# toverainc/willow-inference-server

Measured on AMD Instinct MI355X. Metric: realtime_multiple (audio_ms / infer_ms), Whisper large-v2 beam=5, 3.84 s clip, higher is better.
Workload: dtype f16; 1 GPU; whisper-large beam=5 clip=3sec (3840 ms) batch=1/GPU, PCM resident in HBM -> ids on host; parallelism=1 independent replicas (utterance sharding, no data-path collective)

## Files before the change

### willow-inference-server_amd/csrc/dec_kernels.hip

```cpp
#include <string.h>
#include <atomic>
#include <mutex>
#include "common.hpp"
#include "kernels.hpp"

namespace wis {

__global__ void pack_gemv_kernel(const f16* __restrict__ W, f16* __restrict__ Wp, int N, int Npad, int K, int n_scale, float scale, int rows) {
  const int ksteps = K / 32;
  const size_t total = (size_t)Npad * ksteps * 4;
  for (size_t idx = (size_t)blockIdx.x * blockDim.x + threadIdx.x; idx < total; idx += (size_t)gridDim.x * blockDim.x) {
    const int row = (int)(idx % rows);
    size_t t = idx / rows;
    const int kq = (int)(t & 3); t >>= 2;
    const int ks = (int)(t % ksteps), nt = (int)(t / ksteps);
    const int n = rows * nt + row, k = 32 * ks + 8 * kq;
    f16x8 v;
    if (n < N) {
      v = *reinterpret_cast<const f16x8*>(W + (size_t)n * K + k);
      if (n < n_scale) {
#pragma unroll
        for (int j = 0; j < 8; ++j) v[j] = (f16)((float)v[j] * scale);
      }
    } else {
// ... 1945 lines not shown
    if (pub) {
#pragma unroll
      for (int blk = 0; blk < NB; ++blk)
#pragma unroll
        for (int r4 = 0; r4 < 4; ++r4) own[l15][dhb + 16 * blk + r4] = o_[blk][r4];
      if (wave == NKW && kq == 0) { own[l15][64] = Mc; own[l15][65] = Lc; }
    }
    __syncthreads();
    stamp(pf, 5);
    for (int item = tid; item < R * 32; item += NTHR) {
      const int r = item >> 5, dp = item & 31;
      float2 ml[CM], ov[CM];
      unsigned spins = 0;
      for (;;) {
        bool ok = true;
#pragma unroll
        for (int cc = 0; cc < CM - 1; ++cc) {
          if (cc < C - 1) {
            const gran_t* gp = gbase + ((size_t)cc * 8 + r) * 66;
            const gran_t g0 = ld_gran(gp + 64), g1 = ld_gran(gp + 65), g2 = ld_gran(gp + 2 * dp), g3 = ld_gran(gp + 2 * dp + 1);
            ok = ok & ((unsigned)(g0 >> 32) == tag) & ((unsigned)(g1 >> 32) == tag) & ((unsigned)(g2 >> 32) == tag) & ((unsigned)(g3 >> 32) == tag);
            ml[cc] = make_float2(__uint_as_float((unsigned)g0), __uint_as_float((unsigned)g1));
            ov[cc] = make_float2(__uint_as_float((unsigned)g2), __uint_as_float((unsigned)g3));
          }
        }
        if (ok) break;
        if (++spins > CA_SPIN_LIMIT) { atomicOr(epoch, 1u); break; }
        __builtin_amdgcn_s_sleep(1);
      }
      float M_ = own[r][64];
#pragma unroll
      for (int cc = 0; cc < CM - 1; ++cc) if (cc < C - 1) M_ = fmaxf(M_, ml[cc].x);
      float L = 0.f, O0 = 0.f, O1 = 0.f;
#pragma unroll
      for (int cc = 0; cc < CM - 1; ++cc) {
        if (cc < C - 1) {
          const float w = __expf(ml[cc].x - M_);
          L = fmaf(ml[cc].y, w, L); O0 = fmaf(ov[cc].x, w, O0); O1 = fmaf(ov[cc].y, w, O1);
        }
      }
      {
        const float w = __expf(own[r][64] - M_);
        L = fmaf(own[r][65], w, L); O0 = fmaf(own[r][2 * dp], w, O0); O1 = fmaf(own[r][2 * dp + 1], w, O1);
      }
      const float inv = 1.0f / L;
      typedef _Float16 f16x2 __attribute__((ext_vector_type(2)));
      const f16x2 o2 = {(f16)(O0 * inv), (f16)(O1 * inv)};
      *reinterpret_cast<f16x2*>(out + (out_mb ? xf_index(b * R + r, h * 64 + 2 * dp, out_mb) : (size_t)(b * R + r) * d + h * 64 + 2 * dp)) = o2;
    }
    if (tid == 0) __hip_atomic_store(epoch + 1 + b * H + h, tag, __ATOMIC_RELAXED, __HIP_MEMORY_SCOPE_AGENT);
    stamp(pf, 6);
    if (tid == 0) tl_end(prof);
    return;
  }
  float* pbase = part + ((size_t)(b * H + h) * C) * R * 66;
  if (pub) {
    float* pp = pbase + ((size_t)c * R + l15) * 66;
#pragma unroll
    for (int blk = 0; blk < NB; ++blk)
#pragma unroll
      for (int r4 = 0; r4 < 4; ++r4) st_sc1(pp + dhb + 16 * blk + r4, o_[blk][r4]);
    if (wave == NKW && kq == 0) { st_sc1(pp + 64, Mc); st_sc1(pp + 65, Lc); }
  }
  asm volatile("s_waitcnt vmcnt(0)" ::: "memory");
  __syncthreads();
  stamp(pf, 5);
  if (tid == 0) {
    const unsigned prev = __hip_atomic_fetch_add(counters + b * H + h, 1u, __ATOMIC_RELAXED, __HIP_MEMORY_SCOPE_AGENT);
    const int last = (prev == (unsigned)(C - 1));
    if (last) {
      __hip_atomic_store(counters + b * H + h, 0u, __ATOMIC_RELAXED, __HIP_MEMORY_SCOPE_AGENT);
      __builtin_amdgcn_fence(__ATOMIC_ACQUIRE, "agent");
    }
    s_last = last;
  }
  __syncthreads();
  if (tid == 0) tl_end(prof);
  if (!s_last) return;
  for (int item = tid; item < R * 32; item += NTHR) {
    const int r = item >> 5, dp = item & 31;
    float2 ml[CM], ov[CM];
#pragma unroll
    for (int cc = 0; cc < CM; ++cc) {
      if (cc < C) {
        const float* pp = pbase + ((size_t)cc * R + r) * 66;
        ml[cc] = *reinterpret_cast<const float2*>(pp + 64);
        ov[cc] = *reinterpret_cast<const float2*>(pp + 2 * dp);
      }
    }
    float M_ = -INFINITY;
#pragma unroll
    for (int cc = 0; cc < CM; ++cc) if (cc < C) M_ = fmaxf(M_, ml[cc].x);
    float L = 0.f, O0 = 0.f, O1 = 0.f;
#pragma unroll
    for (int cc = 0; cc < CM; ++cc) {
      if (cc < C) {
        const float w = __expf(ml[cc].x - M_);
        L = fmaf(ml[cc].y, w, L); O0 = fmaf(ov[cc].x, w, O0); O1 = fmaf(ov[cc].y, w, O1);
      }
    }
    const float inv = 1.0f / L;
    typedef _Float16 f16x2 __attribute__((ext_vector_type(2)));
    const f16x2 o2 = {(f16)(O0 * inv), (f16)(O1 * inv)};
    *reinterpret_cast<f16x2*>(out + (out_mb ? xf_index(b * R + r, h * 64 + 2 * dp, out_mb) : (size_t)(b * R + r) * d + h * 64 + 2 * dp)) = o2;
  }
  stamp(pf, 6);
}

int launch_dec_cross_attn(hipStream_t st, const float* q, const f16* kx, const f16* vt, f16* out, float* part, unsigned* counters,
                          int B, int R, int H, int d, int T, int Tpad, int chunks, unsigned long long* prof, int out_mb,
                          const float* xres, const float* qcs, const float* qb, unsigned long long* gran, unsigned* epoch, const float* q2, int xres_is_stat, int kv_shared) {
  if (xres && (!qcs || !qb || R > 8 || d > (xres_is_stat ? 2048 : 1280))) { set_error("dec_cross_attn: folded query needs column sums, bias, R <= 8 and d <= 1280 (2048 from partials)"); return WIS_E_ARG; }
  if (xres_is_stat && !xres) { set_error("dec_cross_attn: the fold from partials needs the row partials"); return WIS_E_ARG; }
  if (R < 1 || R > 16 || chunks < 1 || chunks > 16) { set_error("dec_cross_attn: R=%d chunks=%d unsupported", R, chunks); return WIS_E_UNSUPPORTED; }
  if (H > 63 || d > 65535 || T > 65535) { set_error("dec_cross_attn: H=%d d=%d T=%d beyond the packed shape arguments", H, d, T); return WIS_E_UNSUPPORTED; }
  const int CL = cdiv(cdiv(T, chunks), 32) * 32;
  if ((CL != 128 && CL != 256) || CL * chunks > Tpad) { set_error("dec_cross_attn: %d chunks of %d keys unsupported (Tpad %d)", chunks, CL, Tpad); return WIS_E_UNSUPPORTED; }
  const int used = cdiv(T, CL);
  static const int env_spin = getenv("WIS_CA_SPIN") ? atoi(getenv("WIS_CA_SPIN")) : 1;
  const bool spin = env_spin && gran && epoch && B * H <= CA_SPIN_MAX_BH && CL == 256 && used >= 2 && used <= 6 && R <= 8;
  static const int lds_pad = getenv("WIS_CA_LDS_PAD") ? atoi(getenv("WIS_CA_LDS_PAD")) : 0;
  const int shm = (long)B * H * used > 512 ? lds_pad : 0;
#define WIS_CA(TPWv, CMv, FOLDv, SPINv) hipLaunchKernelGGL((dec_cross_attn_kernel<TPWv, CMv, FOLDv, SPINv>), dim3(used, H, B), dim3(256), shm, st, q, kx, vt, xres, q2, epoch, \
                                                  (R | (H << 8) | (CL << 14) | (used << 24)), (d | (T << 16)), (Tpad | (kv_shared ? (1 << 30) : 0)), out, part, counters, prof, out_mb, qcs, qb, gran)
  if (xres_is_stat) {
    const bool small = (long)B * H * used <= 256;
    static const int ca_rs = getenv("WIS_CA_RS") ? atoi(getenv("WIS_CA_RS")) : 2;
    if (ca_rs && (!small || ca_rs >= 2) && CL == 256 && used <= 6 && R <= 8 && d <= 1280) {
#define WIS_CA_RS(SPINv, NTv, NKWv) hipLaunchKernelGGL((dec_cross_attn_rs_kernel<SPINv, NTv, NKWv>), dim3(used, H, B), dim3(128 * NKWv), 0, st, q, kx, vt, xres, q2, epoch, \
                                                        (R | (H << 8) | (CL << 14) | (used << 24)), (d | (T << 16)), (Tpad | (kv_shared ? (1 << 30) : 0)), out, part, counters, prof, out_mb, qcs, qb, gran)
      static const bool rs8 = getenv("WIS_CA_RS8") && atoi(getenv("WIS_CA_RS8")) != 0;
      if (spin) { if (small && rs8) WIS_CA_RS(true, true, 4); else if (small) WIS_CA_RS(true, true, 2); else WIS_CA_RS(true, false, 2); }
      else { if (small && rs8) WIS_CA_RS(false, true, 4); else if (small) WIS_CA_RS(false, true, 2); else WIS_CA_RS(false, false, 2); }
#undef WIS_CA_RS
      return WIS_OK;
    }
    static const bool fold4 = !(getenv("WIS_CA_FOLD4") && atoi(getenv("WIS_CA_FOLD4")) == 0);
    const bool f4 = fold4 && !small && R <= 8;
    if (spin) { if (small) WIS_CA(4, 6, 3, true); else if (f4) WIS_CA(4, 6, 4, true); else WIS_CA(4, 6, 2, true); }
    else if (CL <= 128) WIS_CA(2, 16, 2, false);
    else if (used <= 6) { if (small) WIS_CA(4, 6, 3, false); else if (f4) WIS_CA(4, 6, 4, false); else WIS_CA(4, 6, 2, false); } else WIS_CA(4, 16, 2, false);
  }
  else if (spin) { if (xres) WIS_CA(4, 6, 1, true); else WIS_CA(4, 6, 0, true); }
  else if (xres) { if (CL <= 128) WIS_CA(2, 16, 1, false); else if (used <= 6) WIS_CA(4, 6, 1, false); else WIS_CA(4, 16, 1, false); }
  else { if (CL <= 128) WIS_CA(2, 16, 0, false); else if (used <= 6) WIS_CA(4, 6, 0, false); else WIS_CA(4, 16, 0, false); }
#undef WIS_CA
  return WIS_OK;
}

__device__ __forceinline__ bool better(float av, int ai, float bv, int bi) { return av > bv || (av == bv && ai < bi); }
__device__ __forceinline__ bool better_b(float av, int ai, float bv, int bi) { return (av > bv) | ((av == bv) & (ai < bi)); }
__device__ __forceinline__ void take_better(float& v, int& i, float ov, int oi) { const bool t = better_b(ov, oi, v, i); v = t ? ov : v; i = t ? oi : i; }

template <bool TS>
__global__ __launch_bounds__(256) void logit_stats_kernel(const float* __restrict__ logits, const float* __restrict__ bias_all,
                                                          const float* __restrict__ bias_begin, const int* __restrict__ step_u,
                                                          float* __restrict__ st_max, float* __restrict__ st_sum,
                                                          float* __restrict__ st_val, int* __restrict__ st_idx, SampleCfg cfg,
                                                          int lr_b, int lr_j, int lr_off, unsigned long long* prof, const int* __restrict__ rowmap,
                                                          const int* __restrict__ ts_desc) {
  constexpr int PT = 16;
  const int tid = threadIdx.x, lane = tid & 63, wave = tid >> 6;
  const int sc = blockIdx.x * 4 + wave, m = blockIdx.y, b = m / cfg.beam;
  unsigned long long* pf = (blockIdx.x == 0 && blockIdx.y == 0 && tid == 0) ? prof : nullptr;
  stamp(pf, 0);
  const int step = step_u[b];
  const int SL = cdiv(cfg.n_vocab, STAT_SUB);
  const int lo = sc * SL, hi = (lo + SL < cfg.n_vocab) ? lo + SL : cfg.n_vocab;
  const int jb = m - b * cfg.beam;
  const float* row = logits + (size_t)(b * lr_b + (rowmap ? rowmap[jb] : jb) * lr_j + lr_off) * cfg.n_vocab_pad;
  const bool first = (step == 0) && cfg.suppress_blank;
  const bool mask_eot = cfg.fixed_new > 0 && step < cfg.fixed_new;
  const bool force_eot = cfg.fixed_new > 0 && step >= cfg.fixed_new;

  float vals[PT]; u64 keys[PT];
  float lv[PT], la[PT], lb[PT];
  int r0l = 0, r0h = 0, r1l = 0, r1h = 0, r2l = 0, r2h = 0;
  if constexpr (TS) {
    const int* dsc = ts_desc + m * TS_DESC_INTS;
    r0l = dsc[0]; r0h = dsc[1]; r1l = dsc[2]; r1h = dsc[3]; r2l = dsc[4]; r2h = dsc[5];
  }
#pragma unroll
  for (int i = 0; i < PT; ++i) {
    const int nidx = lo + lane + 64 * i;
    const int cidx = nidx < hi ? nidx : hi - 1;
    lv[i] = row[cidx]; lb[i] = bias_begin[cidx]; la[i] = bias_all ? bias_all[cidx] : 0.f;
  }
  float mx = -INFINITY;
#pragma unroll
  for (int i = 0; i < PT; ++i) {
    const int nidx = lo + lane + 64 * i;
    float v = lv[i] + la[i];
    v = first ? v + lb[i] : v;
    bool dead = (nidx >= hi) | (mask_eot & (nidx == cfg.eot)) | (force_eot & (nidx != cfg.eot));
    if constexpr (TS) dead = dead | ((nidx >= r0l) & (nidx < r0h)) | ((nidx >= r1l) & (nidx < r1h)) | ((nidx >= r2l) & (nidx < r2h));
    v = dead ? -INFINITY : v;
    vals[i] = v; keys[i] = nidx < hi ? sel_key(v, nidx) : 0ull; mx = fmaxf(mx, v);
  }
  stamp(pf, 1);
  mx = wave_max(mx);
  float sum = 0.f;
  if (mx > -INFINITY) {
#pragma unroll
    for (int i = 0; i < PT; ++i) sum += __expf(vals[i] - mx);
  }
  sum = wave_sum(sum);
  if (lane == 0) { st_max[m * STAT_SUB + sc] = mx; st_sum[m * STAT_SUB + sc] = sum; }
  stamp(pf, 2);
  u64 prev = ~0ull;
  for (int rnd = 0; rnd < cfg.n_cand; ++rnd) {
    u64 t[PT];
#pragma unroll
    for (int i = 0; i < PT; ++i) t[i] = keys[i] < prev ? keys[i] : 0ull;
#pragma unroll
    for (int w = PT / 2; w >= 1; w >>= 1)
#pragma unroll
      for (int i = 0; i < w; ++i) t[i] = key_max(t[i], t[i + w]);
    const u64 best = wave_max_key(t[0]);
    if (lane == 0) {
      st_val[((size_t)m * STAT_SUB + sc) * cfg.n_cand + rnd] = best ? key_value(best) : -INFINITY;
      st_idx[((size_t)m * STAT_SUB + sc) * cfg.n_cand + rnd] = best ? key_index(best) : 0x7fffffff;
    }
    prev = best;
  }
  stamp(pf, 3);
}
int launch_logit_stats(hipStream_t st, const float* logits, const float* bias_all, const float* bias_begin, const int* step_u,
                       float* st_max, float* st_sum, float* st_val, int* st_idx, int B, const SampleCfg& cfg, int lr_b, int lr_j, int lr_off,
                       unsigned long long* prof, const int* rowmap, const int* ts_desc) {
  if (cdiv(cfg.n_vocab, STAT_SUB) > 16 * 64) { set_error("logit_stats: vocab too large"); return WIS_E_UNSUPPORTED; }
  if (ts_desc) hipLaunchKernelGGL(logit_stats_kernel<true>, dim3(STAT_SUB / 4, B * cfg.beam), dim3(256), 0, st, logits, bias_all, bias_begin, step_u,
                                  st_max, st_sum, st_val, st_idx, cfg, lr_b, lr_j, lr_off, prof, rowmap, ts_desc);
  else hipLaunchKernelGGL(logit_stats_kernel<false>, dim3(STAT_SUB / 4, B * cfg.beam), dim3(256), 0, st, logits, bias_all, bias_begin, step_u,
                          st_max, st_sum, st_val, st_idx, cfg, lr_b, lr_j, lr_off, prof, rowmap, nullptr);
  return WIS_OK;
}

__device__ __forceinline__ float block_max_256(float v, float* red) {
  v = wave_max(v);
  const int lane = threadIdx.x & 63, wave = threadIdx.x >> 6;
  __syncthreads();
  if (lane == 0) red[wave] = v;
  __syncthreads();
  return fmaxf(fmaxf(red[0], red[1]), fmaxf(red[2], red[3]));
}
__device__ __forceinline__ float block_sum_256(float v, float* red) {
  v = wave_sum(v);
  const int lane = threadIdx.x & 63, wave = threadIdx.x >> 6;
  __syncthreads();
  if (lane == 0) red[wave] = v;
  __syncthreads();
  return (red[0] + red[1]) + (red[2] + red[3]);
}
__global__ __launch_bounds__(256) void ts_rules_kernel(const float* __restrict__ logits, const float* __restrict__ bias_all,
                                                       const float* __restrict__ bias_begin, const int* __restrict__ step_u,
                                                       const int* __restrict__ alive, SampleCfg cfg, int no_ts, int max_init,
                                                       int lr_b, int lr_j, int lr_off, int* __restrict__ ts_desc) {
  __shared__ float red[4];
  const int tid = threadIdx.x, m = blockIdx.x, b = m / cfg.beam, jb = m - b * cfg.beam;
  const int V = cfg.n_vocab, tb = no_ts + 1;
  int step = step_u[b];
  step = step < cfg.max_new ? step : cfg.max_new;
  const bool force_eot = cfg.fixed_new > 0 && step >= cfg.fixed_new;
  int* dsc = ts_desc + m * TS_DESC_INTS;
  if (force_eot) {
    if (tid < TS_DESC_INTS) dsc[tid] = (tid == 7) ? step : 0;
    return;
  }
  const bool first = (step == 0) && cfg.suppress_blank;
  const bool mask_eot = cfg.fixed_new > 0 && step < cfg.fixed_new;
  int r0l = no_ts, r0h = no_ts + 1, r1l = 0, r1h = 0, r2l = 0, r2h = 0;
  if (step == 0) {
    r0l = 0; r0h = tb;
    if (max_init >= 0 && tb + max_init + 1 < V) { r1l = tb + max_init + 1; r1h = V; }
  } else {
    const int* hist = alive + (size_t)m * cfg.max_new;
    const int tk = tid < step ? hist[tid] : -1;
    const float lastpos = block_max_256(tk >= tb ? (float)tid : -1.f, red);
    const int last = hist[step - 1];
    const bool last_ts = last >= tb;
    const bool pen_ts = step < 2 || hist[step - 2] >= tb;
    if (last_ts) { if (pen_ts) { r1l = tb; r1h = V; } else { r1l = 0; r1h = cfg.eot; } }
    if (lastpos >= 0.f) {
      const int t_ts = hist[(int)lastpos];
      const int t_last = (last_ts && !pen_ts) ? t_ts : t_ts + 1;
      r2l = tb; r2h = t_last;
    }
  }
  const float* row = logits + (size_t)(b * lr_b + jb * lr_j + lr_off) * cfg.n_vocab_pad;
  auto value = [&](int i) -> float {
    float v = row[i] + (bias_all ? bias_all[i] : 0.f);
    v = first ? v + bias_begin[i] : v;
    const bool dead = (mask_eot & (i == cfg.eot)) | ((i >= r0l) & (i < r0h)) | ((i >= r1l) & (i < r1h)) | ((i >= r2l) & (i < r2h));
    return dead ? -INFINITY : v;
  };
  float tmx = -INFINITY;
  for (int i = tid; i < tb; i += 256) tmx = fmaxf(tmx, value(i));
  float smx = -INFINITY;
  for (int i = tb + tid; i < V; i += 256) smx = fmaxf(smx, value(i));
  tmx = block_max_256(tmx, red);
  smx = block_max_256(smx, red);
  float ssum = 0.f;
  if (smx > -INFINITY)
    for (int i = tb + tid; i < V; i += 256) ssum += expf(value(i) - smx);
  ssum = block_sum_256(ssum, red);
  const float lse = smx > -INFINITY ? smx + logf(ssum) : -INFINITY;
  const bool ts_wins = lse > tmx;
  if (ts_wins) { r0l = 0; r0h = tb; }
  if (tid == 0) {
    dsc[0] = r0l; dsc[1] = r0h; dsc[2] = r1l; dsc[3] = r1h; dsc[4] = r2l; dsc[5] = r2h; dsc[6] = ts_wins ? 1 : 0; dsc[7] = step;
  }
}
int launch_ts_rules(hipStream_t st, const float* logits, const float* bias_all, const float* bias_begin, const BeamState& bs, int B,
                    const SampleCfg& cfg, int no_ts, int max_init, int lr_b, int lr_j, int lr_off, int* ts_desc) {
  if (cfg.max_new > 256 || no_ts + 1 >= cfg.n_vocab) { set_error("ts_rules: config out of range"); return WIS_E_UNSUPPORTED; }
  hipLaunchKernelGGL(ts_rules_kernel, dim3(B * cfg.beam), dim3(256), 0, st, logits, bias_all, bias_begin, bs.step_u, bs.alive, cfg, no_ts, max_init,
                     lr_b, lr_j, lr_off, ts_desc);
  return WIS_OK;
}

__global__ __launch_bounds__(256) void no_speech_kernel(const float* __restrict__ logits, int ld, int rs, int r0, int V, int ns, float* __restrict__ out) {
  __shared__ float red[4];
  const int b = blockIdx.x, tid = threadIdx.x;
  const float* row = logits + (size_t)(b * rs + r0) * ld;
  float mx = -INFINITY;
  for (int i = tid; i < V; i += 256) mx = fmaxf(mx, row[i]);
  mx = block_max_256(mx, red);
  float s = 0.f;
  for (int i = tid; i < V; i += 256) s += expf(row[i] - mx);
  s = block_sum_256(s, red);
  if (tid == 0) out[b] = expf(row[ns] - mx) / s;
}
int launch_no_speech(hipStream_t st, const float* logits, int ld, int B, int rs, int r0, int V, int ns, float* out) {
  if (ns < 0 || ns >= V) { set_error("no_speech: token %d outside the vocabulary", ns); return WIS_E_ARG; }
  hipLaunchKernelGGL(no_speech_kernel, dim3(B), dim3(256), 0, st, logits, ld, rs, r0, V, ns, out);
  return WIS_OK;
}

__global__ __launch_bounds__(64) void greedy_pick_kernel(const float* __restrict__ st_max, const float* __restrict__ st_sum, const float* __restrict__ st_val,
                                                         const int* __restrict__ st_idx, int n_cand, int V, int* __restrict__ tok_out, float* __restrict__ lp_out) {
  const int m = blockIdx.x, lane = threadIdx.x;
  const float smx = st_max[m * STAT_SUB + lane], ssm = st_sum[m * STAT_SUB + lane];
  const float v = st_val[((size_t)m * STAT_SUB + lane) * n_cand];
  const int ix = st_idx[((size_t)m * STAT_SUB + lane) * n_cand];
  const float M_ = wave_max(smx);
  const float S = wave_sum(smx > -INFINITY ? ssm * __expf(smx - M_) : 0.f);
  const float lse = M_ + logf(S);
  const int tk = ix > V - 1 ? V - 1 : ix;
  const u64 best = wave_max_key(sel_key(v > -INFINITY ? v - lse : -INFINITY, tk));
  if (lane == 0) { tok_out[m] = key_index(best); lp_out[m] = key_value(best); }
}
int launch_greedy_pick(hipStream_t st, const float* st_max, const float* st_sum, const float* st_val, const int* st_idx, int rows, const SampleCfg& cfg, int* tok_out, float* lp_out) {
  hipLaunchKernelGGL(greedy_pick_kernel, dim3(rows), dim3(64), 0, st, st_max, st_sum, st_val, st_idx, cfg.n_cand, cfg.n_vocab, tok_out, lp_out);
  return WIS_OK;
}

__device__ __forceinline__ void publish_step(const BeamState& bs) {
  __threadfence();
  const unsigned B = gridDim.x;
  const unsigned n = atomicAdd(bs.tick, 1u) + 1u;
  if (n % B != 0u) return;
  __threadfence();
  const unsigned steps = n / B;
  const unsigned done = (unsigned)__hip_atomic_load(bs.all_done, __ATOMIC_RELAXED, __HIP_MEMORY_SCOPE_AGENT);
  const unsigned gen = __hip_atomic_load(bs.tick + 1, __ATOMIC_RELAXED, __HIP_MEMORY_SCOPE_AGENT);
  const unsigned gu = bs.giveup ? (__hip_atomic_load(bs.giveup, __ATOMIC_RELAXED, __HIP_MEMORY_SCOPE_AGENT) != 0u ? 1u : 0u) : 0u;
  const unsigned long long now = (unsigned long long)__builtin_amdgcn_s_memrealtime();
  if (steps == 1u) __hip_atomic_store(bs.host + HP_STAMP0, now, __ATOMIC_RELAXED, __HIP_MEMORY_SCOPE_SYSTEM);
  __hip_atomic_store(bs.host + HP_STAMP, now, __ATOMIC_RELAXED, __HIP_MEMORY_SCOPE_SYSTEM);
  if (done >= B && atomicCAS(bs.tick + 2, 0u, steps) == 0u) {
    __hip_atomic_store(bs.host + HP_DONE_STEP, (unsigned long long)steps, __ATOMIC_RELAXED, __HIP_MEMORY_SCOPE_SYSTEM);
    __hip_atomic_store(bs.host + HP_DONE_STAMP, now, __ATOMIC_RELAXED, __HIP_MEMORY_SCOPE_SYSTEM);
  }
  const unsigned long long rec = ((unsigned long long)(gen & 0xFFFFu) << 48) | ((unsigned long long)(steps & 0xFFFFu) << 32) | ((unsigned long long)gu << 16) | (done & 0xFFFFu);
  __hip_atomic_store(bs.host + HP_REC, rec, __ATOMIC_RELEASE, __HIP_MEMORY_SCOPE_SYSTEM);
}

template <int PSL>
__global__ __launch_bounds__(256) void beam_step_kernel(const float* __restrict__ st_max, const float* __restrict__ st_sum,
                                                        const float* __restrict__ st_val, const int* __restrict__ st_idx,
                                                        BeamState bs, RowMeta rm, int P, int ctx, SampleCfg cfg, unsigned long long* prof) {
  constexpr int HPT = (MAX_R * 256 + 255) / 256;
  __shared__ float lse[MAX_R], s_cum[MAX_R];
  __shared__ float cand_v[MAX_CAND]; __shared__ int cand_word[MAX_CAND]; __shared__ int cand_org[MAX_CAND];
  __shared__ int nb_src[MAX_R]; __shared__ int nb_tok[MAX_R]; __shared__ float nb_cum[MAX_R];
  __shared__ int hyp_src[MAX_R]; __shared__ int hyp_slot[MAX_R]; __shared__ int hyp_n[MAX_R]; __shared__ int n_newhyp;
  __shared__ int s_finished;
  __shared__ int sh_alive[MAX_R * 256];
  const int b = blockIdx.x, tid = threadIdx.x, lane = tid & 63, wave = tid >> 6;
  unsigned long long* pf = (b == 0 && tid == 0) ? prof : nullptr;
  stamp(pf, 0);
  const int k = cfg.beam, NC = cfg.n_cand, V = cfg.n_vocab;
  const int r0 = b * k, per_row = STAT_SUB * NC, total = k * per_row;
  float pv_[PSL]; int pi_[PSL];
#pragma unroll
  for (int u = 0; u < PSL; ++u) {
    const int e = tid + 256 * u, ce = e < total ? e : total - 1;
    const float v = st_val[(size_t)r0 * per_row + ce]; const int ix = st_idx[(size_t)r0 * per_row + ce];
    pv_[u] = e < total ? v : -INFINITY; pi_[u] = e < total ? ix : 0x7fffffff;
  }
  float smx[2], ssm[2];
#pragma unroll
  for (int j2 = 0; j2 < 2; ++j2) {
    const int j = wave + 4 * j2, mrow = r0 + (j < k ? j : 0);
    smx[j2] = st_max[mrow * STAT_SUB + lane]; ssm[j2] = st_sum[mrow * STAT_SUB + lane];
  }
  const float my_cum = tid < k ? bs.cum[r0 + tid] : 0.f;
  int hist_tok[HPT];
#pragma unroll
  for (int u = 0; u < HPT; ++u) {
    const int i = tid + 256 * u, j = i >> 8, t = i & 255;
    const int cj = j < k ? j : k - 1, ct = t < cfg.max_new ? t : cfg.max_new - 1;
    hist_tok[u] = bs.alive[(size_t)(r0 + cj) * cfg.max_new + ct];
  }
  const int done_b = bs.done[b];
  const int step = bs.step_u[b];
  const int nh0 = bs.n_hyp[b];
  if (done_b) { if (tid == 0) publish_step(bs); return; }

  stamp(pf, 1);
#pragma unroll
  for (int u = 0; u < HPT; ++u) { const int i = tid + 256 * u; if (i < MAX_R * 256) sh_alive[i] = hist_tok[u]; }
  if (tid < k) s_cum[tid] = my_cum;
#pragma unroll
  for (int j2 = 0; j2 < 2; ++j2) {
    const int j = wave + 4 * j2;
    const float M_ = wave_max(smx[j2]);
    const float S = wave_sum(smx[j2] > -INFINITY ? ssm[j2] * __expf(smx[j2] - M_) : 0.f);
    if (lane == 0 && j < k) lse[j] = M_ + logf(S);
  }
  __syncthreads();
  stamp(pf, 2);
  u64 pk[PSL];
  u64 lbest = 0ull;
  const float inv_per_row = 1.0f / (float)per_row;
#pragma unroll
  for (int u = 0; u < PSL; ++u) {
    const int e = tid + 256 * u;
    int j = (int)(((float)e + 0.5f) * inv_per_row);
    j = j < k ? j : k - 1;
    const float v = pv_[u];
    const float sc_ = (v - lse[j]) + s_cum[j];
    int tk = pi_[u]; tk = tk > V - 1 ? V - 1 : tk;
    pk[u] = e < total ? sel_key(v > -INFINITY ? sc_ : -INFINITY, (j << 20) | tk) : 0ull;
    lbest = key_max(lbest, pk[u]);
  }
  stamp(pf, 3);
  __shared__ u64 wcand[4 * MAX_CAND];
  for (int rnd = 0; rnd < NC; ++rnd) {
    const u64 wb = wave_max_key(lbest);
    if (lane == 0) wcand[wave * NC + rnd] = wb;
#pragma unroll
    for (int u = 0; u < PSL; ++u) pk[u] = pk[u] == wb ? 0ull : pk[u];
    u64 t[PSL];
#pragma unroll
    for (int u = 0; u < PSL; ++u) t[u] = pk[u];
#pragma unroll
    for (int w = PSL / 2; w >= 1; w >>= 1)
#pragma unroll
      for (int u = 0; u < w; ++u) t[u] = key_max(t[u], t[u + w]);
    lbest = t[0];
  }
  if (tid < MAX_CAND) { cand_v[tid] = -INFINITY; cand_word[tid] = V - 1; cand_org[tid] = 0; }
  __syncthreads();
  if (tid < 4 * NC) {
    const u64 mine = wcand[tid];
    int rank = 0;
#pragma unroll
    for (int m2 = 0; m2 < 4 * MAX_CAND; ++m2) rank += (m2 < 4 * NC && wcand[m2] > mine) ? 1 : 0;
    if (mine != 0ull && rank < NC) {
      const int bi = key_index(mine);
      cand_v[rank] = key_value(mine); cand_word[rank] = bi & 0xFFFFF; cand_org[rank] = (bi >> 20) & 0x7FF;
    }
  }
  __syncthreads();

  stamp(pf, 4);
  if (tid == 0) {
    const bool is_last = (step + 1 >= cfg.max_new);
    int nh = nh0, second = k, newh = 0; bool top_finished = false;
    for (int kk = 0; kk < k; ++kk) {
      int next = kk;
      const bool eos = cand_word[kk] == cfg.eot;
      if (eos || is_last) {
        if (kk == 0) top_finished = true;
        if (nh < cfg.max_hyp) {
          hyp_src[newh] = kk; hyp_slot[newh] = nh; hyp_n[newh] = eos ? step : step + 1;
          bs.hyp_score[b * cfg.max_hyp + nh] = cand_v[kk];
          bs.hyp_len[b * cfg.max_hyp + nh] = hyp_n[newh];
          ++newh; ++nh;
        }
        for (int j = second; j < NC; ++j)
          if (cand_word[j] != cfg.eot) { next = j; second = j + 1; break; }
      }
      nb_src[kk] = next; nb_tok[kk] = cand_word[next]; nb_cum[kk] = cand_v[next];
    }
    n_newhyp = newh;
    bs.n_hyp[b] = nh;
    bool fin = is_last;
    if (!fin) fin = cfg.allow_early_exit ? (top_finished && nh >= cfg.early_exit_hyps) : (nh >= cfg.max_candidates);
    s_finished = fin ? 1 : 0;
  }
  __syncthreads();

  stamp(pf, 5);
  const int hist = step;
  const int npos = P - 1 + step + 1;
  for (int hh = 0; hh < n_newhyp; ++hh) {
    const int kk = hyp_src[hh], org = cand_org[kk], n = hyp_n[hh];
    int* dst = bs.hyp_tok + ((size_t)b * cfg.max_hyp + hyp_slot[hh]) * cfg.max_new;
    for (int t = tid; t < n; t += 256) dst[t] = (t < hist) ? sh_alive[org * 256 + t] : cand_word[kk];
  }
  if (s_finished) {
    __syncthreads();
    __threadfence_block();
    if (tid == 0) {
      const int nh = bs.n_hyp[b];
      int best = 0; float bsc = -INFINITY;
      for (int i = 0; i < nh; ++i) {
        float s = bs.hyp_score[b * cfg.max_hyp + i];
        const int n = bs.hyp_len[b * cfg.max_hyp + i];
        if (cfg.length_penalty != 0.f) s /= powf((float)n, cfg.length_penalty);
        if (s > bsc) { bsc = s; best = i; }
      }
      cand_org[0] = best;
      bs.out_len[b] = bs.hyp_len[b * cfg.max_hyp + best];
      bs.out_score[b] = bsc;
      bs.done[b] = 1;
      hp_out_len(bs.host)[b] = bs.hyp_len[b * cfg.max_hyp + best];
      hp_out_score(bs.host)[b] = bsc;
    }
    __syncthreads();
    const int best = cand_org[0], n = bs.hyp_len[b * cfg.max_hyp + best];
    const int* src = bs.hyp_tok + ((size_t)b * cfg.max_hyp + best) * cfg.max_new;
    int* hids = hp_out_ids(bs.host) + (size_t)b * cfg.max_new;
    for (int t = tid; t < n; t += 256) { const int v = src[t]; bs.out_ids[(size_t)b * cfg.max_new + t] = v; hids[t] = v; }
    __threadfence_system();
    __syncthreads();
    if (tid == 0) { atomicAdd(bs.all_done, 1); publish_step(bs); }
    return;
  }
  stamp(pf, 7);
  for (int j = 0; j < k; ++j) {
    const int org = cand_org[nb_src[j]];
    int* al = bs.alive + (size_t)(r0 + j) * cfg.max_new;
    for (int t = tid; t < hist; t += 256) al[t] = sh_alive[org * 256 + t];
    if (tid == 0) {
      al[hist] = nb_tok[j];
      bs.parent[r0 + j] = (step == 0) ? r0 : r0 + org;
      { int* tr = bs.traj + ((size_t)(b * 256 + step) * MAX_R + j) * 2; tr[0] = nb_tok[j]; tr[1] = org; }
      bs.cum[r0 + j] = nb_cum[j];
      rm.tok[r0 + j] = nb_tok[j];
      rm.pos[r0 + j] = npos;
      rm.slot[r0 + j] = r0 + j;
    }
  }
  if (tid == 0) bs.step_u[b] = step + 1;
  __syncthreads();
  if (tid == 0) publish_step(bs);
  stamp(pf, 8);
}
int launch_beam_step(hipStream_t st, const float* st_max, const float* st_sum, const float* st_val, const int* st_idx,
                     const BeamState& bs, const RowMeta& rm, int B, int P, int ctx, const SampleCfg& cfg, unsigned long long* prof) {
  if (cfg.beam > MAX_R || cfg.n_cand > MAX_CAND || cfg.max_new > 256 || ctx > 512 || cfg.n_vocab > (1 << 20)) { set_error("beam_step: config out of range"); return WIS_E_UNSUPPORTED; }
  if (cfg.beam * STAT_SUB * cfg.n_cand <= 16 * 256) hipLaunchKernelGGL(beam_step_kernel<16>, dim3(B), dim3(256), 0, st, st_max, st_sum, st_val, st_idx, bs, rm, P, ctx, cfg, prof);
  else hipLaunchKernelGGL(beam_step_kernel<32>, dim3(B), dim3(256), 0, st, st_max, st_sum, st_val, st_idx, bs, rm, P, ctx, cfg, prof);
  return WIS_OK;
}

constexpr int VS_PERM = 8, VS_BASE = 16, VS_PATH = 32, VS_PATH_W = 32, VS_INTS = VS_PATH + MAX_R * VS_PATH_W;
__global__ __launch_bounds__(64) void draft_match_kernel(BeamState bs, const int* __restrict__ draft, int n_draft, int k, int* __restrict__ vs, int book) {
  __shared__ int org_r[MAX_R], tok_r[MAX_R], perm_prev[MAX_R], old_base[MAX_R], old_path[MAX_R][VS_PATH_W];
  const int tid = threadIdx.x;
  if (bs.done[0]) return;
  const int s = bs.step_u[0] - 1;
  const int t = vs[2];
  if (tid < k) {
    const int* tr = bs.traj + ((size_t)s * MAX_R + tid) * 2;
    tok_r[tid] = tr[0]; org_r[tid] = tr[1]; perm_prev[tid] = vs[VS_PERM + tid]; old_base[tid] = vs[VS_BASE + tid];
  }
  for (int e = tid; e < k * VS_PATH_W; e += 64) old_path[e / VS_PATH_W][e % VS_PATH_W] = vs[VS_PATH + e];
  __syncthreads();
  if (book) {
    for (int e = tid; e < k * VS_PATH_W; e += 64) {
      const int j = e / VS_PATH_W, u = e % VS_PATH_W, pj = org_r[j];
      if (u < t) vs[VS_PATH + e] = old_path[pj][u];
      else if (u == t) vs[VS_PATH + e] = perm_prev[pj];
    }
    if (tid < k) vs[VS_BASE + tid] = old_base[org_r[tid]];
  }
  if (tid == 0) {
    bool ok = s >= 0 && s < n_draft;
    int pn[MAX_R]; unsigned used = 0;
    if (ok) {
      const int* dr = draft + (size_t)s * MAX_R * 2;
      for (int j = 0; j < k && ok; ++j) {
        const int want_org = perm_prev[org_r[j]];
        int hit = -1;
        for (int i = 0; i < k; ++i) if (!((used >> i) & 1u) && dr[2 * i] == tok_r[j] && dr[2 * i + 1] == want_org) { hit = i; break; }
        if (hit < 0) ok = false; else { pn[j] = hit; used |= 1u << hit; }
      }
    }
    if (ok) { for (int j = 0; j < k; ++j) vs[VS_PERM + j] = pn[j]; vs[0] = s + 1; }
    else bs.done[0] = 2;
    if (book) vs[2] = t + 1;
  }
}
int launch_draft_match(hipStream_t st, const BeamState& bs, const int* draft, int n_draft, int beam, int* vstate, int book) {
  hipLaunchKernelGGL(draft_match_kernel, dim3(1), dim3(64), 0, st, bs, draft, n_draft, beam, vstate, book);
  return WIS_OK;
}
__global__ __launch_bounds__(256) void kv_gather_kernel(f16* __restrict__ kc, f16* __restrict__ vc, size_t lstride, const int* __restrict__ vs, const int* __restrict__ done,
                                                        int k, int w0, int ctx, int d) {
  const int lk = blockIdx.y, tid = threadIdx.x;
  const int nwin = vs[2];
  if (done[0] == 1 || nwin <= 0) return;
  f16* cache = ((lk & 1) ? vc : kc) + (size_t)(lk >> 1) * lstride;
  const int c8 = d >> 3, npos = w0 + nwin;
  for (int p = blockIdx.x; p < npos; p += gridDim.x) {
    int par[MAX_R];
#pragma unroll
    for (int j = 0; j < MAX_R; ++j) par[j] = j < k ? (p < w0 ? vs[VS_BASE + j] : vs[VS_PATH + j * VS_PATH_W + (p - w0)]) : j;
    for (int ch = tid; ch < c8; ch += 256) {
      u32x4 v[MAX_R];
#pragma unroll
      for (int j = 0; j < MAX_R; ++j) if (j < k && par[j] != j) v[j] = *reinterpret_cast<const u32x4*>(cache + ((size_t)par[j] * ctx + p) * d + ch * 8);
      asm volatile("s_waitcnt vmcnt(0)" ::: "memory");
#pragma unroll
      for (int j = 0; j < MAX_R; ++j) if (j < k && par[j] != j) *reinterpret_cast<u32x4*>(cache + ((size_t)j * ctx + p) * d + ch * 8) = v[j];
    }
  }
}
int launch_kv_gather(hipStream_t st, f16* kc, f16* vc, size_t layer_stride, int L, const int* vstate, const int* done, int beam, int w0, int ctx, int d) {
  hipLaunchKernelGGL(kv_gather_kernel, dim3(8, 2 * L), dim3(256), 0, st, kc, vc, layer_stride, vstate, done, beam, w0, ctx, d);
  return WIS_OK;
}

__global__ __launch_bounds__(256) void kv_reorder_kernel(f16* __restrict__ kc, f16* __restrict__ vc, size_t lstride, const int* __restrict__ parent,
                                                         const int* __restrict__ step_u, const int* __restrict__ done, int k, int P, int ctx, int d) {
  const int b = blockIdx.z, lk = blockIdx.y, tid = threadIdx.x;
  if (k < 2) return;
  const int r0 = b * k;
  const int dn = done[b], st = step_u[b];
  int par[MAX_R];
#pragma unroll
  for (int j = 0; j < MAX_R; ++j) par[j] = parent[r0 + (j < k ? j : 0)];
  bool ident = true;
#pragma unroll
  for (int j = 0; j < MAX_R; ++j) { if (j < k) ident = ident & (par[j] == r0 + j); else par[j] = r0 + j; }
  if (dn | (int)ident) return;
  const int npos = P - 1 + st;
  f16* cache = ((lk & 1) ? vc : kc) + (size_t)(lk >> 1) * lstride;
  const int c8 = d >> 3;
  for (int p = blockIdx.x; p < npos; p += gridDim.x) {
    for (int ch = tid; ch < c8; ch += 256) {
      u32x4 v[MAX_R];
#pragma unroll
      for (int j = 0; j < MAX_R; ++j) if (j < k && par[j] != r0 + j) v[j] = *reinterpret_cast<const u32x4*>(cache + ((size_t)par[j] * ctx + p) * d + ch * 8);
      asm volatile("s_waitcnt vmcnt(0)" ::: "memory");
#pragma unroll
      for (int j = 0; j < MAX_R; ++j) if (j < k && par[j] != r0 + j) *reinterpret_cast<u32x4*>(cache + ((size_t)(r0 + j) * ctx + p) * d + ch * 8) = v[j];
    }
  }
}
int launch_kv_reorder(hipStream_t st, f16* kc, f16* vc, size_t layer_stride, int L, const BeamState& bs, int B, int beam, int P, int ctx, int d) {
  if (beam < 2) return WIS_OK;
  if (beam > MAX_R) { set_error("kv_reorder: beam %d > %d", beam, MAX_R); return WIS_E_UNSUPPORTED; }
  hipLaunchKernelGGL(kv_reorder_kernel, dim3(8, 2 * L, B), dim3(256), 0, st, kc, vc, layer_stride, bs.parent, bs.step_u, bs.done, beam, P, ctx, d);
  return WIS_OK;
}

__global__ void lang_probs_kernel(const float* __restrict__ logits, int ld, const int* __restrict__ lang_ids, int n_lang, float* __restrict__ probs) {
  const int b = blockIdx.x, lane = threadIdx.x;
  const float* row = logits + (size_t)b * ld;
  float mx = -INFINITY;
  for (int i = lane; i < n_lang; i += 64) mx = fmaxf(mx, row[lang_ids[i]]);
  mx = wave_max(mx);
  float s = 0.f;
  for (int i = lane; i < n_lang; i += 64) s += __expf(row[lang_ids[i]] - mx);
  s = wave_sum(s);
  for (int i = lane; i < n_lang; i += 64) probs[(size_t)b * n_lang + i] = __expf(row[lang_ids[i]] - mx) / s;
}
int launch_lang_probs(hipStream_t st, const float* logits, int ld, const int* lang_ids, int n_lang, float* probs, int B) {
  hipLaunchKernelGGL(lang_probs_kernel, dim3(B), dim3(64), 0, st, logits, ld, lang_ids, n_lang, probs);
  return WIS_OK;
}

}
```

### willow-inference-server_amd/csrc/kernels.hpp

```cpp
#pragma once
#include "common.hpp"

namespace wis {

struct GemmP {
  const f16* A; int64_t a_bs; int a_rs; int a_rpb;
  const f16* W;
  int M, N, K;
  int klen;
  int n_span = 0, n_period = 0, n_phase = 0;
};
static inline GemmP gemm_plain(const f16* A, int lda, const f16* W, int M, int N, int K) {
  GemmP p; p.A = A; p.a_bs = 0; p.a_rs = lda; p.a_rpb = 0x7fffffff; p.W = W; p.M = M; p.N = N; p.K = K; p.klen = 0; return p;
}
int launch_layernorm(hipStream_t st, const float* x, const float* gamma, const float* beta, f16* y, int M, int d);
int launch_gemm_generic(hipStream_t st, const GemmP& p, const float* bias, const float* resid, void* C, int flags);
int launch_gemm_splitk_resid(hipStream_t st, const GemmP& p, int splits, float* scratch, const float* bias, const float* resid, float* X,
                             const float* ln_gamma = nullptr, const float* ln_beta = nullptr, f16* Y = nullptr);
int launch_gemm_conv1(hipStream_t st, const GemmP& p, const float* bias, f16* C, int T);
int launch_gemm_conv2(hipStream_t st, const GemmP& p, const float* bias, const float* pos, float* X, int T);
int launch_gemm_qkv(hipStream_t st, const GemmP& p, const float* bias, f16* qk, f16* vt, int d, int T, int Tpad, int H);
int launch_gemm_crosskv(hipStream_t st, const GemmP& p, const float* bias, f16* kx, f16* vt, int d, int T, int Tpad, int H, int64_t kx_lstride, int64_t vt_lstride);
int launch_enc_attention(hipStream_t st, const f16* qk, const f16* vt, f16* out, int B, int T, int Tpad, int H, float* part = nullptr, unsigned* counters = nullptr,
                         size_t part_cap = 0);
size_t enc_attention_part_floats(int B, int T, int H);
bool enc_attn_lazy();
void launch_scale_q_log2e(hipStream_t st, f16* qk, int64_t rows, int d);

constexpr int MAX_ROWS = 96;
constexpr int MAX_R = 8;
constexpr int MAX_CAND = 2 * MAX_R;
constexpr int MAX_HYP = 3 * MAX_R;

struct RowMeta {
  int* tok;
  int* pos;
  int* slot;
  int* lslot;
};

enum { GV_GELU = 1, GV_RESID = 2, GV_OUT_F32 = 4, GV_LN = 8, GV_QKV = 16,
       GV_LNP = 32,
       GV_LN16 = 64 };
struct GemvP {
  const void* x;
  const float* gamma; const float* beta;
  const float* csum;
  const f16* Wp; const float* bias;
  const float* wscale;
  void* y;
  int M, N, K, flags;
  float* q; f16* kc; f16* vc; const int* slot; const int* pos; int d; int ctx;
  unsigned long long* prof;
  int rows;
  const void* x2; int xsplit;
  f16* y16;
  int xmb;
  const float* stat_in;
  float* stat_out;
  f16* y_xf;
  int ymb;
  int ksplit; float* kpart; unsigned* kcnt;
  int mb0, mbi;
  int wks, wk0;
  unsigned long long* sa_gran; unsigned* sa_epoch; unsigned* sa_flag; f16* sa_out; int sa_rpu, sa_sstride, sa_first;
};
int launch_gemv(hipStream_t st, const GemvP& p);
int launch_gemv_dual(hipStream_t st, const GemvP& pa, const GemvP& pb, const f16* pf_k = nullptr, const f16* pf_v = nullptr, int pf_T = 0, int pf_Tpad = 0, int pf_chunks = 0, int pf_H = 0);
int launch_gemv_frag(hipStream_t st, const GemvP& p);
int launch_gemv_frag3(hipStream_t st, const GemvP* p, int n);
__host__ __device__ static inline size_t xf_index(int m, int k, int MB) {
  return ((size_t)((k >> 5) * MB + (m >> 4)) * 64 + (m & 15) + 16 * ((k >> 3) & 3)) * 8 + (k & 7);
}
int launch_xf_pack(hipStream_t st, const void* x, int x_f16, f16* xf, float* stat, int M, int K, int MB);
int launch_dec_embed_xf(hipStream_t st, const f16* emb, const f16* pos_emb, const int* tok, const int* pos, float* x, f16* xf, float* stat, int M, int d, int MB);
int launch_fold_ln(hipStream_t st, f16* W, const float* gamma, const float* beta, float* bias, float* csum, int N, int K, int n_scale, float qscale);
int launch_csum8(hipStream_t st, const f16* W, const float* scale, float* csum, int N, int K, int n_scale, float qscale);
int launch_pack_gemv8(hipStream_t st, const f16* W, unsigned char* Wp, float* scale, int N, int Npad, int K, int n_scale, float qscale);
int launch_pack_gemv(hipStream_t st, const f16* W, f16* Wp, int N, int Npad, int K, int n_scale, float scale, int rows = 16);
int gemv_rows_for(int N, int K);

int launch_dec_embed(hipStream_t st, const f16* emb, const f16* pos_emb, const int* tok, const int* pos, float* x, int M, int d, f16* xh = nullptr, float* stat = nullptr);
int launch_dec_self_attn(hipStream_t st, const float* q, const f16* kc, const f16* vc, const int* pos, f16* out,
                         int M, int H, int d, int ctx, int rpu, int sstride, int rmul, unsigned long long* prof = nullptr, int out_mb = 0,
                         const int* anc = nullptr, int w0 = 0, int aw = 0, const int* base = nullptr, int nb = 8);
constexpr int CA_SPIN_MAX_BH = 192;
int launch_dec_cross_attn(hipStream_t st, const float* q, const f16* kx, const f16* vt, f16* out, float* part, unsigned* counters,
                          int B, int R, int H, int d, int T, int Tpad, int chunks, unsigned long long* prof = nullptr, int out_mb = 0,
                          const float* xres = nullptr, const float* qcs = nullptr, const float* qb = nullptr,
                          unsigned long long* gran = nullptr, unsigned* epoch = nullptr,
                          const float* q2 = nullptr, int xres_is_stat = 0,
                          int kv_shared = 0);

struct SampleCfg {
  int n_vocab, n_vocab_pad, eot, beam, n_cand, max_new, fixed_new, suppress_blank, greedy;
  float length_penalty; int max_hyp; int allow_early_exit; int max_candidates;
  int early_exit_hyps;
};
#ifndef WIS_EARLY_EXIT_NUM_HYPOTHESES
#define WIS_EARLY_EXIT_NUM_HYPOTHESES 1
#endif
constexpr int STAT_SUB = 64;
int launch_logit_stats(hipStream_t st, const float* logits, const float* bias_all, const float* bias_begin, const int* step_u,
                       float* st_max, float* st_sum, float* st_val, int* st_idx, int B, const SampleCfg& cfg,
                       int lr_b, int lr_j, int lr_off, unsigned long long* prof = nullptr,
                       const int* rowmap = nullptr,
                       const int* ts_desc = nullptr);
constexpr int TS_DESC_INTS = 8;
struct BeamState;
int launch_ts_rules(hipStream_t st, const float* logits, const float* bias_all, const float* bias_begin, const BeamState& bs, int B,
                    const SampleCfg& cfg, int no_ts, int max_init, int lr_b, int lr_j, int lr_off, int* ts_desc);
int launch_no_speech(hipStream_t st, const float* logits, int ld, int B, int rs, int r0, int V, int ns, float* out);
struct BeamState {
  int* step_u;
  int* done;
  int* n_hyp;
  float* cum;
  int* alive;
  int* parent;
  float* hyp_score;
  int* hyp_len;
  int* hyp_tok;
  int* all_done;
  int* out_ids; int* out_len; float* out_score;
  unsigned* tick;
  const unsigned* giveup;
  unsigned long long* host;
  int* traj;
};
enum { HP_REC = 0,
       HP_STAMP0 = 1,
       HP_STAMP = 2,
       HP_DONE_STEP = 3,
       HP_DONE_STAMP = 4,
       HP_WORDS = 8,
       HP_MAXB = MAX_ROWS };
constexpr size_t HP_BYTES = HP_WORDS * 8 + (size_t)HP_MAXB * 8 + (size_t)HP_MAXB * 256 * 4;
__host__ __device__ inline int* hp_out_len(unsigned long long* hp) { return reinterpret_cast<int*>(hp + HP_WORDS); }
__host__ __device__ inline float* hp_out_score(unsigned long long* hp) { return reinterpret_cast<float*>(hp + HP_WORDS) + HP_MAXB; }
__host__ __device__ inline int* hp_out_ids(unsigned long long* hp) { return reinterpret_cast<int*>(hp + HP_WORDS) + 2 * HP_MAXB; }
int launch_kv_reorder(hipStream_t st, f16* kc, f16* vc, size_t layer_stride, int L, const BeamState& bs, int B, int beam, int P, int ctx, int d);
int launch_beam_step(hipStream_t st, const float* st_max, const float* st_sum, const float* st_val, const int* st_idx,
                     const BeamState& bs, const RowMeta& rm, int B, int P, int ctx, const SampleCfg& cfg, unsigned long long* prof = nullptr);
constexpr int DRAFT_VS_INTS = 32 + MAX_R * 32, DRAFT_VS_PERM = 8, DRAFT_VS_BASE = 16;
int launch_draft_match(hipStream_t st, const BeamState& bs, const int* draft, int n_draft, int beam, int* vstate, int book);
int launch_kv_gather(hipStream_t st, f16* kc, f16* vc, size_t layer_stride, int L, const int* vstate, const int* done, int beam, int w0, int ctx, int d);
int launch_greedy_pick(hipStream_t st, const float* st_max, const float* st_sum, const float* st_val, const int* st_idx, int rows, const SampleCfg& cfg, int* tok_out, float* lp_out);
int launch_lang_probs(hipStream_t st, const float* logits, int ld, const int* lang_ids, int n_lang, float* probs, int B);

}
```

### willow-inference-server_amd/csrc/model.hip

```cpp
#include <math.h>
#include <stdlib.h>
#include <string.h>
#include <time.h>
#include <algorithm>
#include <atomic>
#include <chrono>
#include <map>
#include <mutex>
#include <memory>
#include <string>
#include <vector>

#include "common.hpp"
#include "kernels.hpp"

using namespace wis;

namespace wis {

__global__ void convert_kernel(const void* __restrict__ src, int src_f16, void* __restrict__ dst, int dst_f16,
                               int64_t rows, int64_t cols, int64_t dst_ld, int64_t n_scale, float scale) {
  const int64_t total = rows * cols;
  for (int64_t i = (int64_t)blockIdx.x * blockDim.x + threadIdx.x; i < total; i += (int64_t)gridDim.x * blockDim.x) {
    const int64_t r = i / cols, c = i - r * cols;
    float v = src_f16 ? (float)reinterpret_cast<const f16*>(src)[i] : reinterpret_cast<const float*>(src)[i];
    if (r < n_scale) v *= scale;
    if (dst_f16) reinterpret_cast<f16*>(dst)[r * dst_ld + c] = (f16)v; else reinterpret_cast<float*>(dst)[r * dst_ld + c] = v;
  }
}
__global__ void conv_pack_kernel(const void* __restrict__ src, int src_f16, f16* __restrict__ dst, int out, int in, int cpad, int row_len) {
  const int64_t total = (int64_t)out * row_len;
  for (int64_t i = (int64_t)blockIdx.x * blockDim.x + threadIdx.x; i < total; i += (int64_t)gridDim.x * blockDim.x) {
    const int o = (int)(i / row_len), rem = (int)(i - (int64_t)o * row_len), k = rem / cpad, c = rem - k * cpad;
    float v = 0.f;
    if (k < 3 && c < in) {
      const int64_t s = ((int64_t)o * in + c) * 3 + k;
      v = src_f16 ? (float)reinterpret_cast<const f16*>(src)[s] : reinterpret_cast<const float*>(src)[s];
    }
    dst[i] = (f16)v;
  }
}
template <int NM, int CC>
__global__ void mel_to_image_kernel(const float* __restrict__ mel, f16* __restrict__ img) {
  __shared__ float s_t[NM][65];
  const int tid = threadIdx.x, w = blockIdx.y, f0 = blockIdx.x * 64;
  for (int o = tid; o < NM * 64; o += 256) {
    const int m = o >> 6, f = o & 63;
    if (f0 + f < 3000) s_t[m][f] = mel[((size_t)w * NM + m) * 3000 + f0 + f];
  }
  __syncthreads();
  for (int o = tid; o < 64 * CC; o += 256) {
    const int f = o / CC, c = o - f * CC;
    if (f0 + f < 3000) img[((size_t)w * 3002 + f0 + f + 1) * CC + c] = (c < NM) ? (f16)s_t[c][f] : (f16)0.f;
  }
}
static int conv1_k(int n_mels) { return cdiv(3 * conv1_channels(n_mels), 64) * 64; }
__global__ void transpose_to_f16_kernel(const void* __restrict__ src, int src_f16, f16* __restrict__ dst, int rows, int cols) {
  __shared__ float t[32][33];
  const int c0 = blockIdx.x * 32, r0 = blockIdx.y * 32, tx = threadIdx.x & 31, ty = threadIdx.x >> 5;
  for (int i = ty; i < 32; i += 8) {
    const int r = r0 + i, c = c0 + tx;
    if (r < rows && c < cols) t[i][tx] = src_f16 ? (float)reinterpret_cast<const f16*>(src)[(size_t)r * cols + c] : reinterpret_cast<const float*>(src)[(size_t)r * cols + c];
  }
  __syncthreads();
  for (int i = ty; i < 32; i += 8) {
    const int c = c0 + i, r = r0 + tx;
    if (r < rows && c < cols) dst[(size_t)c * rows + r] = (f16)t[tx][i];
  }
}
__global__ void matvec_rows_kernel(const f16* __restrict__ W, int ld, const float* __restrict__ x, float* __restrict__ y, int N, int K) {
  const int n = blockIdx.x, lane = threadIdx.x;
  if (n >= N) return;
  float a = 0.f;
  for (int k = lane; k < K; k += 64) a += (float)W[(size_t)n * ld + k] * x[k];
  a = wave_sum(a);
  if (lane == 0) y[n] = a;
}
__global__ void f16_to_f32_kernel(const f16* __restrict__ s, float* __restrict__ d, int64_t n) {
  for (int64_t i = (int64_t)blockIdx.x * blockDim.x + threadIdx.x; i < n; i += (int64_t)gridDim.x * blockDim.x) d[i] = (float)s[i];
}
}

struct EncLayerW {
  float *ln1_g, *ln1_b, *ln2_g, *ln2_b;
  f16 *w_qkv, *w_out, *w_f1, *w_f2;
  float *b_qkv, *b_out, *b_f1, *b_f2;
};
struct DecLayerW {
  float *ln1_g, *ln1_b, *ln2_g, *ln2_b, *ln3_g, *ln3_b;
  f16 *p_qkv, *p_out, *p_cq, *p_cout, *p_f1, *p_f2;
  f16 *w_ckv;
  float *b_qkv, *b_out, *b_cq, *b_ckv, *b_cout, *b_f1, *b_f2;
  float *s_qkv = nullptr, *s_out = nullptr, *s_cq = nullptr, *s_cout = nullptr, *s_f1 = nullptr, *s_f2 = nullptr;
  float *c_qkv = nullptr, *c_cq = nullptr, *c_f1 = nullptr;
  f16* p_cqo = nullptr; float* b_cqo = nullptr;
};

struct GraphKey {
  int B, beam, P, max_new, fixed_new, suppress_blank, suppress_default, early_exit, spin, sa_nb; float lp, patience;
  int timestamps, max_init;
  bool operator<(const GraphKey& o) const { return memcmp(this, &o, sizeof(GraphKey)) < 0; }
};

struct WeightSlabs {
  int device; std::vector<void*> slabs; size_t bytes = 0;
  ~WeightSlabs() { hipSetDevice(device); for (void* p : slabs) hipFree(p); }
};

struct AlignState {
  std::vector<int> heads;
  bool ready = false;
  bool capture = false;
  int nsel = 0, sel_cap = 0; size_t sel_bytes = 0;
  std::vector<int> layer_s0;
  int* d_sel_head = nullptr; long long* d_koff = nullptr;
  f16* qsel = nullptr;
  float *W = nullptr, *acc = nullptr;
  unsigned* trace = nullptr; int *rev = nullptr, *path = nullptr, *d_meta = nullptr; float* probs = nullptr;
  int cap_ub0 = 0, cap_t0 = 0, cap_P = 0, last_nmax = 0;
  int kv_ub0 = 0;
  hipEvent_t ev[5 + 128] = {}; int n_ev = 0;
  bool ev_partial = false;
};

struct wis_model {
  wis_config_t cfg;
  int device;
  DeviceCtx* ctx;
  hipStream_t st;
  std::shared_ptr<WeightSlabs> wslabs;
  std::vector<void*> allocs;
  char* slab_cur = nullptr; size_t slab_left = 0;
  size_t bytes = 0;
  f16 *w_conv1, *w_conv2; float *b_conv1, *b_conv2, *enc_pos, *enc_ln_g, *enc_ln_b;
  std::vector<EncLayerW> enc;
  std::vector<DecLayerW> dec;
  f16 *emb, *dec_pos, *p_proj; float *dec_ln_g, *dec_ln_b;
  float *bias_all, *bias_begin; int* d_lang_ids;
  int n_vocab_pad;
  int Tpad;
  f16 *img, *c1, *xn, *qk, *vt, *ao, *hbuf, *mem;
  float* x; float* skbuf; float* enc_part = nullptr; unsigned* enc_cnt = nullptr;
  std::vector<f16*> kx, vx;
  std::vector<f16*> kc, vc;
  f16 *kc_all = nullptr, *vc_all = nullptr; size_t kv_layer_stride = 0;
  f16 *kx_all = nullptr, *vx_all = nullptr, *w_ckv_all = nullptr; float* b_ckv_all = nullptr;
  size_t kx_lstride = 0, vx_lstride = 0;
  float *dx, *dq, *logits, *part; f16 *dao, *dh, *dln; unsigned* counters;
  float* dq2 = nullptr;
  int sa_nb = 8;
  float* gf_part = nullptr; unsigned* gf_cnt = nullptr; int gf_ksplit = 1;
  unsigned long long* ca_gran = nullptr; unsigned* ca_epoch = nullptr;
  unsigned long long* sa_gran = nullptr; unsigned* sa_epoch = nullptr;
  bool spin_off = false;
  int handoff_retries = 0;
  bool spin_now = true;
  f16 *dxf = nullptr, *daoxf = nullptr, *dhxf = nullptr; float* dstat = nullptr;
  RowMeta rm; BeamState bs;
  RowMeta rm_win;
  float *st_max, *st_sum, *st_val; int* st_idx;
  int* ts_desc = nullptr;
  float* d_nsp = nullptr;
  int nsp_B = 0;
  float* d_in; int64_t* d_nsamp; float* d_probs;
  int* vstep = nullptr; int* pick_tok = nullptr; float* pick_lp = nullptr;
  int* d_draft = nullptr; int* d_anc = nullptr; int* d_vstate = nullptr; int* d_base = nullptr;
  float* lm_logspec = nullptr; unsigned* lm_gmax = nullptr;
  int* h_pin;
  unsigned long long* h_prog = nullptr;
  unsigned gen = 0;
  int last_B = 0, last_beam = 0;
  bool overrun_left = false;
  hipEvent_t ev[8];
  hipStream_t st_enc = nullptr;
  hipEvent_t ev_enc = nullptr, ev_ckv = nullptr;
  wis_timing_t timing;
  std::map<GraphKey, hipGraphExec_t> graphs;
  bool use_graph;
  float* s_proj = nullptr;
  float* c_proj = nullptr; float* b_proj = nullptr;
  bool w8 = false;
  bool cq_fold = false;
  f16* dxh = nullptr;
  unsigned long long* d_prof;
  bool prof_on; bool prof_all;
  size_t enc_part_cap = 0;
  std::atomic_flag busy = ATOMIC_FLAG_INIT;
  AlignState al;
};

namespace {

constexpr size_t SLAB_BYTES = (size_t)1 << 30;
static int enc_splitk(int d, int M) {
  const int tiles = (d / 128) * cdiv(M, 128);
  if (tiles >= 200) return 0;
  return (tiles <= 128 && (4 * d) % (4 * 64) == 0) ? 4 : 2;
}
template <class T>
int dalloc(wis_model* m, T** p, size_t n_elems) {
  size_t b = n_elems * sizeof(T); if (b == 0) b = 16;
  const size_t align = b >= ((size_t)1 << 20) ? ((size_t)1 << 16) : 256;
  size_t pad = (align - (reinterpret_cast<uintptr_t>(m->slab_cur) & (align - 1))) & (align - 1);
  if (!m->slab_cur || pad + b > m->slab_left) {
    const size_t sb = b > SLAB_BYTES ? ((b + ((size_t)2 << 20) - 1) & ~(((size_t)2 << 20) - 1)) : SLAB_BYTES;
    void* q = nullptr;
    hipError_t e = hipMalloc(&q, sb);
    if (e != hipSuccess) { set_error("hipMalloc(%zu bytes) failed: %s", sb, hipGetErrorString(e)); return WIS_E_NOMEM; }
    m->allocs.push_back(q); m->slab_cur = static_cast<char*>(q); m->slab_left = sb; pad = 0;
  }
  m->slab_cur += pad; m->slab_left -= pad;
  *p = reinterpret_cast<T*>(m->slab_cur);
  m->slab_cur += b; m->slab_left -= b; m->bytes += b + pad;
  return WIS_OK;
}
inline int blocks_for(int64_t n) { int64_t b = (n + 255) / 256; return (int)(b > 8192 ? 8192 : (b < 1 ? 1 : b)); }

struct TensorSrc { const void* p; int f16; int64_t rows, cols; };

struct Loader {
  const wis_tensor_t* t; int n; const char* arena;
  size_t arena_bytes;
  const wis_tensor_t* find(const std::string& name) const {
    for (int i = 0; i < n; ++i) if (name == t[i].name) return &t[i];
    return nullptr;
  }
  int get(const std::string& name, int64_t rows, int64_t cols, TensorSrc* out) const {
    const wis_tensor_t* x = find(name);
    if (!x) { set_error("weight '%s' missing from the index", name.c_str()); return WIS_E_FORMAT; }
    int64_t ne = 1; for (int i = 0; i < x->rank; ++i) ne *= x->shape[i];
    if (ne != rows * cols) { set_error("weight '%s': %lld elements, expected %lld", name.c_str(), (long long)ne, (long long)(rows * cols)); return WIS_E_FORMAT; }
    const size_t es = x->dtype == WIS_DT_F16 ? 2 : 4;
    if (x->dtype != WIS_DT_F16 && x->dtype != WIS_DT_F32) { set_error("weight '%s': dtype %d unsupported", name.c_str(), x->dtype); return WIS_E_FORMAT; }
    if (x->offset + (size_t)ne * es > arena_bytes) { set_error("weight '%s' exceeds the arena", name.c_str()); return WIS_E_FORMAT; }
    out->p = arena + x->offset; out->f16 = x->dtype == WIS_DT_F16; out->rows = rows; out->cols = cols;
    return WIS_OK;
  }
};

int to_f32(wis_model* m, const Loader& L, const std::string& name, int64_t n, float** out, int64_t n_scale = 0, float scale = 1.f) {
  TensorSrc s; WIS_RET(L.get(name, n, 1, &s));
  if (!*out) WIS_RET(dalloc(m, out, (size_t)n));
  hipLaunchKernelGGL(convert_kernel, dim3(blocks_for(n)), dim3(256), 0, m->st, s.p, s.f16, *out, 0, n, (int64_t)1, (int64_t)1, n_scale, scale);
  return WIS_OK;
}
int to_f16_mat(wis_model* m, const Loader& L, const std::string& name, int64_t rows, int64_t cols, f16** out, int64_t n_scale = 0, float scale = 1.f) {
  TensorSrc s; WIS_RET(L.get(name, rows, cols, &s));
  if (!*out) WIS_RET(dalloc(m, out, (size_t)rows * cols));
  hipLaunchKernelGGL(convert_kernel, dim3(blocks_for(rows * cols)), dim3(256), 0, m->st, s.p, s.f16, *out, 1, rows, cols, cols, n_scale, scale);
  return WIS_OK;
}
int to_packed(wis_model* m, const Loader& L, const std::string& name, int N, int K, f16** out, f16* tmp, int n_scale = 0, float scale = 1.f, int* npad_out = nullptr,
              float** scale_out = nullptr, const float* ln_gamma = nullptr, const float* ln_beta = nullptr, float* bias = nullptr, float** csum_out = nullptr) {
  TensorSrc s; WIS_RET(L.get(name, N, K, &s));
  const int rows = gemv_rows_for(N, K);
  const int Npad = cdiv(N, rows) * rows;
  hipLaunchKernelGGL(convert_kernel, dim3(blocks_for((int64_t)N * K)), dim3(256), 0, m->st, s.p, s.f16, tmp, 1, (int64_t)N, (int64_t)K, (int64_t)K, (int64_t)0, 1.f);
  if (ln_gamma) {
    if (!bias || !csum_out) { set_error("to_packed: LayerNorm folding needs a bias vector and a column-sum output"); return WIS_E_ARG; }
    WIS_RET(dalloc(m, csum_out, (size_t)Npad));
    WIS_HIP_CHECK(hipMemsetAsync(*csum_out, 0, (size_t)Npad * 4, m->st));
    WIS_RET(launch_fold_ln(m->st, tmp, ln_gamma, ln_beta, bias, *csum_out, N, K, n_scale, scale));
  }
  if (m->w8 && scale_out) {
    unsigned char* q8 = nullptr;
    WIS_RET(dalloc(m, &q8, (size_t)Npad * K));
    WIS_RET(dalloc(m, scale_out, (size_t)Npad));
    WIS_RET(launch_pack_gemv8(m->st, tmp, q8, *scale_out, N, Npad, K, n_scale, scale));
    if (ln_gamma) WIS_RET(launch_csum8(m->st, tmp, *scale_out, *csum_out, N, K, n_scale, scale));
    *out = reinterpret_cast<f16*>(q8);
  } else {
    WIS_RET(dalloc(m, out, (size_t)Npad * K));
    WIS_RET(launch_pack_gemv(m->st, tmp, *out, N, Npad, K, n_scale, scale, rows));
  }
  if (npad_out) *npad_out = Npad;
  return WIS_OK;
}

int load_weights(wis_model* m, const Loader& L) {
  const wis_config_t& c = m->cfg;
  const int d = c.d_model, V = c.n_vocab;
  const float qs = 0.125f;
  f16* tmp = nullptr;
  f16 *fcat = nullptr, *fwot = nullptr, *fwqo = nullptr;
  {
    size_t big = (size_t)V * d; if ((size_t)4 * d * d > big) big = (size_t)4 * d * d;
    WIS_HIP_CHECK(hipMalloc(reinterpret_cast<void**>(&tmp), big * 2));
    if (m->cq_fold) {
      WIS_HIP_CHECK(hipMalloc(reinterpret_cast<void**>(&fcat), (size_t)2 * d * d * 2));
      WIS_HIP_CHECK(hipMalloc(reinterpret_cast<void**>(&fwot), (size_t)d * d * 2));
      WIS_HIP_CHECK(hipMalloc(reinterpret_cast<void**>(&fwqo), (size_t)d * d * 2));
    }
  }
  int rc = WIS_OK;
  do {
    {
      TensorSrc s;
      if ((rc = L.get("encoder/conv1/weight", d, (int64_t)c.n_mels * 3, &s))) break;
      const int cc = conv1_channels(c.n_mels), k1 = conv1_k(c.n_mels);
      if ((rc = dalloc(m, &m->w_conv1, (size_t)d * k1))) break;
      hipLaunchKernelGGL(conv_pack_kernel, dim3(blocks_for((int64_t)d * k1)), dim3(256), 0, m->st, s.p, s.f16, m->w_conv1, d, c.n_mels, cc, k1);
      if ((rc = L.get("encoder/conv2/weight", d, (int64_t)d * 3, &s))) break;
      if ((rc = dalloc(m, &m->w_conv2, (size_t)d * 3 * d))) break;
      hipLaunchKernelGGL(conv_pack_kernel, dim3(blocks_for((int64_t)d * 3 * d)), dim3(256), 0, m->st, s.p, s.f16, m->w_conv2, d, d, d, 3 * d);
    }
    if ((rc = to_f32(m, L, "encoder/conv1/bias", d, &m->b_conv1))) break;
    if ((rc = to_f32(m, L, "encoder/conv2/bias", d, &m->b_conv2))) break;
    if (L.find("encoder/position_encodings/encodings")) {
      if ((rc = to_f32(m, L, "encoder/position_encodings/encodings", (int64_t)c.n_audio_ctx * d, &m->enc_pos))) break;
    } else {
      std::vector<float> pe((size_t)c.n_audio_ctx * d);
      const int half = d / 2; const double inc = log(10000.0) / (half - 1);
      for (int t = 0; t < c.n_audio_ctx; ++t)
        for (int i = 0; i < half; ++i) {
          const float inv = (float)exp(-inc * i);
          const float a = (float)t * inv;
          pe[(size_t)t * d + i] = sinf(a); pe[(size_t)t * d + half + i] = cosf(a);
        }
      if ((rc = dalloc(m, &m->enc_pos, pe.size()))) break;
      WIS_HIP_CHECK(hipMemcpyAsync(m->enc_pos, pe.data(), pe.size() * 4, hipMemcpyHostToDevice, m->st));
      WIS_HIP_CHECK(hipStreamSynchronize(m->st));
    }
    if ((rc = to_f32(m, L, "encoder/layer_norm/gamma", d, &m->enc_ln_g))) break;
    if ((rc = to_f32(m, L, "encoder/layer_norm/beta", d, &m->enc_ln_b))) break;
    m->enc.resize(c.n_enc_layers);
    for (int l = 0; l < c.n_enc_layers && !rc; ++l) {
      const std::string p = "encoder/layer_" + std::to_string(l) + "/";
      EncLayerW& w = m->enc[l];
      if ((rc = to_f32(m, L, p + "self_attention/layer_norm/gamma", d, &w.ln1_g))) break;
      if ((rc = to_f32(m, L, p + "self_attention/layer_norm/beta", d, &w.ln1_b))) break;
      const float qs_enc = enc_attn_lazy() ? qs * 1.4426950408889634f : qs;
// ... 250 lines not shown
}
int run_cross_kv(wis_model* m, int B) {
  const wis_config_t& c = m->cfg;
  const int d = c.d_model, T = c.n_audio_ctx;
  return launch_gemm_crosskv(m->st, gemm_plain(m->mem, d, m->w_ckv_all, B * T, c.n_dec_layers * 2 * d, d), m->b_ckv_all, m->kx_all, m->vx_all, d, T, m->Tpad,
                             c.n_heads, (int64_t)m->kx_lstride, (int64_t)m->vx_lstride);
}

static int launch_ln_gemv(wis_model* m, hipStream_t st, GemvP g) {
  if (g.M > 8 && (g.flags & GV_LN)) {
    WIS_RET(launch_layernorm(st, reinterpret_cast<const float*>(g.x), nullptr, nullptr, m->dln, g.M, g.K));
    g.x = m->dln; g.csum = nullptr; g.flags &= ~GV_LN;
  }
  return launch_gemv(st, g);
}

static inline void cpu_relax() {
#if !defined(__HIP_DEVICE_COMPILE__) && defined(__x86_64__)
  __builtin_ia32_pause();
#endif
}
static std::atomic<int> g_spin_bh[64];
struct DeferredClaim { hipEvent_t ev; int n; };
static std::mutex g_spin_mu;
static std::vector<DeferredClaim> g_spin_deferred[64];
static void spin_collect(int device) {
  std::lock_guard<std::mutex> lk(g_spin_mu);
  auto& v = g_spin_deferred[device & 63];
  for (size_t i = 0; i < v.size();) {
    if (hipEventQuery(v[i].ev) != hipErrorNotReady) { g_spin_bh[device & 63].fetch_sub(v[i].n, std::memory_order_relaxed); v[i] = v.back(); v.pop_back(); }
    else ++i;
  }
}
struct SpinClaim {
  wis_model* m; int n = 0;
  SpinClaim(wis_model* mm, int B) : m(mm) {
    static const bool env_share = getenv("WIS_CA_SPIN_SHARED") != nullptr;
    m->spin_now = false;
    spin_collect(m->device);
    if (m->spin_off) return;
    if (env_share) { m->spin_now = true; return; }
    const int need = B * m->cfg.n_heads;
    std::atomic<int>& a = g_spin_bh[m->device & 63];
    int cur = a.load(std::memory_order_relaxed);
    while (cur + need <= CA_SPIN_MAX_BH)
      if (a.compare_exchange_weak(cur, cur + need, std::memory_order_relaxed)) { n = need; m->spin_now = true; return; }
  }
  ~SpinClaim() { if (n) g_spin_bh[m->device & 63].fetch_sub(n, std::memory_order_relaxed); }
  void defer(hipStream_t st) {
    if (!n) return;
    if (hipEventRecord(m->ev[6], st) != hipSuccess) return;
    std::lock_guard<std::mutex> lk(g_spin_mu);
    auto& v = g_spin_deferred[m->device & 63];
    for (auto& d : v) if (d.ev == m->ev[6]) { d.n += n; n = 0; return; }
    v.push_back({m->ev[6], n}); n = 0;
  }
  SpinClaim(const SpinClaim&) = delete;
  SpinClaim& operator=(const SpinClaim&) = delete;
};
static int spin_gave_up(wis_model* m, bool* gave_up) {
  int* h = m->h_pin + 2;
  WIS_HIP_CHECK(hipMemcpyAsync(h, m->ca_epoch, 4, hipMemcpyDeviceToHost, m->st));
  WIS_HIP_CHECK(hipStreamSynchronize(m->st));
  *gave_up = *h != 0;
  if (*gave_up) {
    WIS_HIP_CHECK(hipMemsetAsync(m->ca_epoch, 0, 4, m->st));
    m->spin_off = true; ++m->handoff_retries;
    fprintf(stderr, "[wis_hip] device %d: decoder cross-attention granule hand-off timed out; this handle uses the ticket hand-off from now on, the call is repeated\n", m->device);
  }
  return WIS_OK;
}

struct TreeWin { const int* anc; int w0, aw; const int* base = nullptr; };
int align_capture_q(wis_model* m, int l, int M);
constexpr int ANC_W = 32;
static int dec_forward_frag(wis_model* m, int M, int R, int B, bool want_logits, int sstride, int rmul, int chunks, const TreeWin* tw = nullptr) {
  const wis_config_t& c = m->cfg; hipStream_t st = m->st;
  const int d = c.d_model, H = c.n_heads, T = c.n_audio_ctx, ctx = c.n_text_ctx, MB = cdiv(M, 16);
  if (tw && (M % 16 != 0 || R != 16 || B != M / 16)) { set_error("dec_forward_frag: a tree window takes whole groups of 16 rows"); return WIS_E_ARG; }
  WIS_RET(launch_dec_embed_xf(st, m->emb, m->dec_pos, m->rm.tok, m->rm.pos, m->dx, m->dxf, m->dstat, M, d, MB));
  static const bool no_frag_fold = getenv("WIS_NO_FRAG_FOLD") != nullptr;
  const bool fold = m->cq_fold && !no_frag_fold && R <= 8;
  auto base = [&](const void* x, const f16* Wp, const float* wscale, const float* bias, int N, int K, int flags) {
    GemvP g; memset(&g, 0, sizeof(g));
    g.x = x; g.Wp = Wp; g.wscale = wscale; g.bias = bias; g.M = M; g.N = N; g.K = K; g.flags = flags; g.xmb = MB; g.rows = 16;
    return g;
  };
  for (int l = 0; l < c.n_dec_layers; ++l) {
    const DecLayerW& w = m->dec[l];
    unsigned long long* pr = (m->prof_on && l == 0) ? m->d_prof : nullptr;
    GemvP g = base(m->dxf, w.p_qkv, w.s_qkv, w.b_qkv, 3 * d, d, GV_LN | GV_QKV);
    g.csum = w.c_qkv; g.stat_in = m->dstat; g.q = m->dq; g.kc = m->kc[l]; g.vc = m->vc[l]; g.slot = m->rm.slot; g.pos = m->rm.pos; g.d = d; g.ctx = ctx;
    g.prof = pr;
    WIS_RET(launch_gemv_frag(st, g));
    WIS_RET(launch_dec_self_attn(st, m->dq, m->kc[l], m->vc[l], m->rm.pos, m->daoxf, M, H, d, ctx, R, sstride, rmul, nullptr, MB, tw ? tw->anc : nullptr, tw ? tw->w0 : 0, tw ? tw->aw : 0, tw ? tw->base : nullptr, m->sa_nb));
    if (fold) {
      if (m->al.capture) { set_error("dec_forward_frag: an alignment pass needs the un-folded route (more than 8 rows per utterance)"); return WIS_E_STATE; }
      GemvP g3[3];
      g3[0] = base(m->daoxf, w.p_out, nullptr, w.b_out, d, d, GV_RESID);
      g3[0].y = m->dx; g3[0].ymb = MB; g3[0].stat_out = m->dstat; g3[0].prof = pr ? pr + 32 : nullptr;
      g3[1] = base(m->dxf, w.p_cqo, nullptr, w.b_cqo, d, d, GV_OUT_F32);
      g3[1].y = m->dq; g3[1].wks = 2 * d / 32; g3[1].wk0 = 0;
      g3[2] = base(m->daoxf, w.p_cqo, nullptr, nullptr, d, d, GV_OUT_F32);
      g3[2].y = m->dq2; g3[2].wks = 2 * d / 32; g3[2].wk0 = d / 32;
      WIS_RET(launch_gemv_frag3(st, g3, 3));
      WIS_RET(launch_dec_cross_attn(st, m->dq, m->kx[l], m->vx[l], m->daoxf, m->part, m->counters, B, R, H, d, T, m->Tpad, chunks, pr ? pr + 64 : nullptr, MB, m->dstat, w.c_cq, w.b_cq,
                                    m->spin_now ? m->ca_gran : nullptr, m->ca_epoch, m->dq2, 1));
    } else {
    g = base(m->daoxf, w.p_out, w.s_out, w.b_out, d, d, GV_RESID);
    g.y = m->dx; g.y_xf = m->dxf; g.ymb = MB; g.stat_out = m->dstat;
    WIS_RET(launch_gemv_frag(st, g));
    g = base(m->dxf, w.p_cq, w.s_cq, w.b_cq, d, d, GV_LN | GV_OUT_F32);
    g.csum = w.c_cq; g.stat_in = m->dstat; g.y = m->dq;
    WIS_RET(launch_gemv_frag(st, g));
    const size_t ku = (size_t)m->al.kv_ub0 * H * T * 64, vu = (size_t)m->al.kv_ub0 * H * 64 * m->Tpad;
    WIS_RET(launch_dec_cross_attn(st, m->dq, m->kx[l] + ku, m->vx[l] + vu, m->daoxf, m->part, m->counters, B, R, H, d, T, m->Tpad, chunks, nullptr, MB, nullptr, nullptr, nullptr,
                                  (m->spin_now && !tw) ? m->ca_gran : nullptr, m->ca_epoch, nullptr, 0, tw ? 1 : 0));
    if (m->al.capture) WIS_RET(align_capture_q(m, l, M));
    }
    g = base(m->daoxf, w.p_cout, w.s_cout, w.b_cout, d, d, GV_RESID);
    g.y = m->dx; g.y_xf = m->dxf; g.ymb = MB; g.stat_out = m->dstat; g.prof = pr ? pr + 80 : nullptr;
    WIS_RET(launch_gemv_frag(st, g));
    g = base(m->dxf, w.p_f1, w.s_f1, w.b_f1, 4 * d, d, GV_LN | GV_GELU);
    g.csum = w.c_f1; g.stat_in = m->dstat; g.y = m->dhxf; g.ymb = MB; g.prof = pr ? pr + 96 : nullptr;
    WIS_RET(launch_gemv_frag(st, g));
    g = base(m->dhxf, w.p_f2, w.s_f2, w.b_f2, d, 4 * d, GV_RESID);
    g.y = m->dx; g.y_xf = m->dxf; g.ymb = MB; g.stat_out = m->dstat; g.prof = pr ? pr + 112 : nullptr;
    if (m->gf_ksplit > 1 && (4 * d / 32) % (4 * m->gf_ksplit) == 0) { g.ksplit = m->gf_ksplit; g.kpart = m->gf_part; g.kcnt = m->gf_cnt; }
    WIS_RET(launch_gemv_frag(st, g));
  }
  if (want_logits) {
    GemvP g = base(m->dxf, m->p_proj, m->s_proj, m->b_proj, m->n_vocab_pad, d, GV_LN | GV_OUT_F32);
    g.csum = m->c_proj; g.stat_in = m->dstat; g.y = m->logits;
    WIS_RET(launch_gemv_frag(st, g));
  }
  return WIS_OK;
}

static bool sa_fuse_enabled() { const char* e = getenv("WIS_SA_FUSE"); return e && atoi(e) != 0; }
int dec_forward(wis_model* m, int M, int R, int B, bool want_logits, int sstride, int rmul, const TreeWin* tw = nullptr) {
  const wis_config_t& c = m->cfg; hipStream_t st = m->st;
  const int d = c.d_model, H = c.n_heads, T = c.n_audio_ctx, ctx = c.n_text_ctx;
  static const int env_chunks = getenv("WIS_CROSS_CHUNKS") ? atoi(getenv("WIS_CROSS_CHUNKS")) : 0;
  const int chunks = env_chunks ? env_chunks : 6;
  static const bool no_frag = getenv("WIS_NO_FRAG") != nullptr;
  if (tw) return dec_forward_frag(m, M, R, B, want_logits, sstride, rmul, chunks, tw);
  if (M > 8 && !no_frag) return dec_forward_frag(m, M, R, B, want_logits, sstride, rmul, chunks);
  if (m->al.capture) { set_error("wis_align needs the batched-row decoder route (more than 8 rows per pass, WIS_NO_FRAG unset)"); return WIS_E_STATE; }
  const bool fold = m->cq_fold && M <= 8;
  static const int ln_form = [] { const char* e = getenv("WIS_B1_LN"); return !e ? 0 : (!strcmp(e, "f16") ? 2 : (!strcmp(e, "partials") ? 1 : 0)); }();
  const bool ln_ok = fold && d % 64 == 0 && M * (d / 8) <= 13 * 256;
  const bool sa_fuse = m->spin_now && sa_fuse_enabled() && rmul == 1 && M <= 8 && !m->w8 && d % 64 == 0 && ctx >= 64 && !m->prof_on;
  const bool lnp = ln_ok && ln_form == 1 && d <= 1280, ln16 = ln_ok && ln_form == 2 && d <= 2048;
  WIS_RET(launch_dec_embed(st, m->emb, m->dec_pos, m->rm.tok, m->rm.pos, m->dx, M, d, fold ? m->dxh : nullptr, lnp ? m->dstat : nullptr));
  for (int l = 0; l < c.n_dec_layers; ++l) {
    const DecLayerW& w = m->dec[l];
    unsigned long long* pr = (m->prof_on && (l == 0 || m->prof_all)) ? m->d_prof + (size_t)l * 8 * 16 : nullptr;
    GemvP g; memset(&g, 0, sizeof(g));
    g.x = m->dx; g.csum = w.c_qkv; g.Wp = w.p_qkv; g.wscale = w.s_qkv; g.bias = w.b_qkv; g.M = M; g.N = 3 * d; g.K = d;
    g.flags = GV_LN | GV_QKV; g.q = m->dq; g.kc = m->kc[l]; g.vc = m->vc[l]; g.slot = m->rm.slot; g.pos = m->rm.pos; g.d = d; g.ctx = ctx;
    g.prof = pr;
    if (lnp) { g.x = m->dxh; g.stat_in = m->dstat; g.flags = GV_LNP | GV_QKV; }
    if (ln16) { g.x = m->dxh; g.flags = GV_LN16 | GV_QKV; }
    g.rows = gemv_rows_for(g.N == m->n_vocab_pad ? m->cfg.n_vocab : g.N, g.K);
    if (sa_fuse && !lnp && !ln16) { g.sa_gran = m->sa_gran; g.sa_epoch = m->sa_epoch; g.sa_flag = m->ca_epoch; g.sa_out = m->dao; g.sa_rpu = R; g.sa_sstride = sstride; }
    WIS_RET(launch_ln_gemv(m, st, g));
    if (!g.sa_gran) WIS_RET(launch_dec_self_attn(st, m->dq, m->kc[l], m->vc[l], m->rm.pos, m->dao, M, H, d, ctx, R, sstride, rmul, pr ? pr + 16 : nullptr, 0, nullptr, 0, 0, nullptr, m->sa_nb));
    if (fold) {
      GemvP ga; memset(&ga, 0, sizeof(ga));
      ga.x = m->dao; ga.Wp = w.p_out; ga.bias = w.b_out; ga.y = m->dx; ga.M = M; ga.N = d; ga.K = d; ga.flags = GV_RESID; ga.prof = pr ? pr + 32 : nullptr;
      static const bool stat_rows = getenv("WIS_B1_STAT_ROWS") != nullptr;
      if (!stat_rows) ga.stat_out = m->dstat;
      GemvP gb; memset(&gb, 0, sizeof(gb));
      gb.x = m->dxh; gb.x2 = m->dao; gb.xsplit = d; gb.Wp = w.p_cqo; gb.bias = w.b_cqo; gb.y = m->dq; gb.M = M; gb.N = d; gb.K = 2 * d; gb.flags = GV_OUT_F32;
      static const bool ca_pf = getenv("WIS_CA_PREFETCH") && atoi(getenv("WIS_CA_PREFETCH")) != 0;
      if (ca_pf && B == 1) WIS_RET(launch_gemv_dual(st, ga, gb, m->kx[l], m->vx[l], T, m->Tpad, chunks, H));
      else
      WIS_RET(launch_gemv_dual(st, ga, gb));
      if (!stat_rows) WIS_RET(launch_dec_cross_attn(st, m->dq, m->kx[l], m->vx[l], m->dao, m->part, m->counters, B, R, H, d, T, m->Tpad, chunks, pr ? pr + 64 : nullptr, 0,
                                                    m->dstat, w.c_cq, w.b_cq, m->spin_now ? m->ca_gran : nullptr, m->ca_epoch, nullptr, 1));
      else
      WIS_RET(launch_dec_cross_attn(st, m->dq, m->kx[l], m->vx[l], m->dao, m->part, m->counters, B, R, H, d, T, m->Tpad, chunks, pr ? pr + 64 : nullptr, 0,
                                    m->dx, w.c_cq, w.b_cq, m->spin_now ? m->ca_gran : nullptr, m->ca_epoch));
    } else {
    memset(&g, 0, sizeof(g));
    g.x = m->dao; g.Wp = w.p_out; g.wscale = w.s_out; g.bias = w.b_out; g.y = m->dx; g.M = M; g.N = d; g.K = d; g.flags = GV_RESID; g.prof = pr ? pr + 32 : nullptr;
    g.rows = gemv_rows_for(g.N == m->n_vocab_pad ? m->cfg.n_vocab : g.N, g.K);
    WIS_RET(launch_ln_gemv(m, st, g));
    memset(&g, 0, sizeof(g));
    g.x = m->dx; g.csum = w.c_cq; g.Wp = w.p_cq; g.wscale = w.s_cq; g.bias = w.b_cq; g.y = m->dq; g.M = M; g.N = d; g.K = d; g.flags = GV_LN | GV_OUT_F32; g.prof = pr ? pr + 48 : nullptr;
    g.rows = gemv_rows_for(g.N == m->n_vocab_pad ? m->cfg.n_vocab : g.N, g.K);
    WIS_RET(launch_ln_gemv(m, st, g));
    WIS_RET(launch_dec_cross_attn(st, m->dq, m->kx[l], m->vx[l], m->dao, m->part, m->counters, B, R, H, d, T, m->Tpad, chunks, pr ? pr + 64 : nullptr, 0, nullptr, nullptr, nullptr,
                                  m->spin_now ? m->ca_gran : nullptr, m->ca_epoch));
    }
    memset(&g, 0, sizeof(g));
    g.x = m->dao; g.Wp = w.p_cout; g.wscale = w.s_cout; g.bias = w.b_cout; g.y = m->dx; g.M = M; g.N = d; g.K = d; g.flags = GV_RESID; g.prof = pr ? pr + 80 : nullptr;
    if (lnp) { g.y16 = m->dln; g.stat_out = m->dstat; }
    if (ln16) g.y16 = m->dln;
    g.rows = gemv_rows_for(g.N == m->n_vocab_pad ? m->cfg.n_vocab : g.N, g.K);
    WIS_RET(launch_ln_gemv(m, st, g));
    memset(&g, 0, sizeof(g));
    g.x = m->dx; g.csum = w.c_f1; g.Wp = w.p_f1; g.wscale = w.s_f1; g.bias = w.b_f1; g.y = m->dh; g.M = M; g.N = 4 * d; g.K = d; g.flags = GV_LN | GV_GELU; g.prof = pr ? pr + 96 : nullptr;
    if (lnp) { g.x = m->dln; g.stat_in = m->dstat; g.flags = GV_LNP | GV_GELU; }
    if (ln16) { g.x = m->dln; g.flags = GV_LN16 | GV_GELU; }
    g.rows = gemv_rows_for(g.N == m->n_vocab_pad ? m->cfg.n_vocab : g.N, g.K);
    WIS_RET(launch_ln_gemv(m, st, g));
    memset(&g, 0, sizeof(g));
    g.x = m->dh; g.Wp = w.p_f2; g.wscale = w.s_f2; g.bias = w.b_f2; g.y = m->dx; g.M = M; g.N = d; g.K = 4 * d; g.flags = GV_RESID; g.prof = pr ? pr + 112 : nullptr;
    g.y16 = fold ? m->dxh : nullptr;
    if (lnp) g.stat_out = m->dstat;
    g.rows = gemv_rows_for(g.N == m->n_vocab_pad ? m->cfg.n_vocab : g.N, g.K);
    WIS_RET(launch_ln_gemv(m, st, g));
  }
  if (want_logits) {
    GemvP g; memset(&g, 0, sizeof(g));
    g.x = m->dx; g.csum = m->c_proj; g.bias = m->b_proj; g.Wp = m->p_proj; g.wscale = m->s_proj; g.y = m->logits; g.M = M; g.N = m->n_vocab_pad; g.K = d; g.flags = GV_LN | GV_OUT_F32;
    if (lnp) { g.x = m->dxh; g.stat_in = m->dstat; g.flags = GV_LNP | GV_OUT_F32; }
    if (ln16) { g.x = m->dxh; g.flags = GV_LN16 | GV_OUT_F32; }
    g.rows = gemv_rows_for(g.N == m->n_vocab_pad ? m->cfg.n_vocab : g.N, g.K);
    WIS_RET(launch_ln_gemv(m, st, g));
  }
  return WIS_OK;
}

static int init_beam_state(wis_model* m, int B, int beam) {
  hipStream_t st = m->st;
  const int Mrows = B * beam;
  float* cum = reinterpret_cast<float*>(m->h_pin + 2048);
  for (int r = 0; r < Mrows; ++r) cum[r] = (r % beam == 0) ? 0.f : -INFINITY;
  unsigned* tk = reinterpret_cast<unsigned*>(m->h_pin + 2048 + MAX_ROWS);
  m->gen = (m->gen % 0xFFFFu) + 1u;
  tk[0] = 0; tk[1] = m->gen; tk[2] = 0; tk[3] = 0;
  WIS_HIP_CHECK(hipMemcpyAsync(m->bs.cum, cum, (size_t)Mrows * 4, hipMemcpyHostToDevice, st));
  WIS_HIP_CHECK(hipMemcpyAsync(m->bs.tick, tk, 16, hipMemcpyHostToDevice, st));
  WIS_HIP_CHECK(hipMemsetAsync(m->bs.step_u, 0, (size_t)B * 4, st));
  WIS_HIP_CHECK(hipMemsetAsync(m->bs.done, 0, (size_t)B * 4, st));
  WIS_HIP_CHECK(hipMemsetAsync(m->bs.n_hyp, 0, (size_t)B * 4, st));
  WIS_HIP_CHECK(hipMemsetAsync(m->bs.all_done, 0, 16, st));
  WIS_HIP_CHECK(hipMemsetAsync(m->bs.out_len, 0, (size_t)B * 4, st));
  return WIS_OK;
}
static SampleCfg make_sample_cfg(const wis_model* m, const wis_gen_opts_t* o, int beam, int max_new, float* patience_out) {
  const wis_config_t& c = m->cfg;
  SampleCfg sc; memset(&sc, 0, sizeof(sc));
  sc.n_vocab = c.n_vocab; sc.n_vocab_pad = m->n_vocab_pad; sc.eot = c.eot; sc.beam = beam; sc.n_cand = 2 * beam; sc.max_new = max_new;
  sc.fixed_new = o->fixed_new_tokens; sc.suppress_blank = o->suppress_blank; sc.greedy = beam == 1;
  sc.length_penalty = o->length_penalty; sc.max_hyp = MAX_HYP;
  const float patience = o->patience > 0.f ? o->patience : 1.f;
  sc.max_candidates = (int)lroundf((float)beam * patience); if (sc.max_candidates < 1) sc.max_candidates = 1;
  sc.allow_early_exit = (patience == 1.f && o->length_penalty == 0.f) ? 1 : 0;
  sc.early_exit_hyps = WIS_EARLY_EXIT_NUM_HYPOTHESES ? 1 : sc.max_candidates;
  *patience_out = patience;
  return sc;
}

static int check_patience(int beam, float patience) {
  const float p = patience > 0.f ? patience : 1.f;
  const long want = lroundf((float)beam * p);
  if (want > MAX_HYP - beam + 1) {
    set_error("patience %.3g at beam_size %d needs %ld finished hypotheses; the engine holds %d (patience <= %.3g at this beam)", (double)p, beam, want, MAX_HYP - beam + 1,
              (double)(MAX_HYP - beam + 1) / (double)beam);
    return WIS_E_ARG;
  }
  return WIS_OK;
}

int upload_rows(wis_model* m, const std::vector<int>& tok, const std::vector<int>& pos, const std::vector<int>& slot, const std::vector<int>& lslot, bool wait = true, int stage = 1024) {
  const size_t n = tok.size();
  int* h = m->h_pin + stage;
  memcpy(h, tok.data(), n * 4); memcpy(h + MAX_ROWS, pos.data(), n * 4); memcpy(h + 2 * MAX_ROWS, slot.data(), n * 4); memcpy(h + 3 * MAX_ROWS, lslot.data(), n * 4);
  WIS_HIP_CHECK(hipMemcpyAsync(m->rm.tok, h, n * 4, hipMemcpyHostToDevice, m->st));
  WIS_HIP_CHECK(hipMemcpyAsync(m->rm.pos, h + MAX_ROWS, n * 4, hipMemcpyHostToDevice, m->st));
  WIS_HIP_CHECK(hipMemcpyAsync(m->rm.slot, h + 2 * MAX_ROWS, n * 4, hipMemcpyHostToDevice, m->st));
  WIS_HIP_CHECK(hipMemcpyAsync(m->rm.lslot, h + 3 * MAX_ROWS, n * 4, hipMemcpyHostToDevice, m->st));
  if (wait) WIS_HIP_CHECK(hipStreamSynchronize(m->st));
  return WIS_OK;
}

int check_batch(wis_model* m, int B, int beam) {
  if (B < 1 || B > m->cfg.max_batch) { set_error("batch %d outside [1, max_batch=%d]", B, m->cfg.max_batch); return WIS_E_STATE; }
  if (beam < 1 || beam > m->cfg.max_beam || beam > MAX_R) { set_error("beam_size %d outside [1, %d]", beam, m->cfg.max_beam < MAX_R ? m->cfg.max_beam : MAX_R); return WIS_E_STATE; }
  if (B * beam > MAX_ROWS) { set_error("B*beam = %d exceeds %d decoder rows per device batch", B * beam, MAX_ROWS); return WIS_E_STATE; }
  return WIS_OK;
}

static std::atomic<int> g_active_calls[64];
struct BusyGuard {
  wis_model* m; bool ok;
  explicit BusyGuard(wis_model* mm) : m(mm), ok(!mm->busy.test_and_set(std::memory_order_acquire)) { if (ok) g_active_calls[m->device & 63].fetch_add(1, std::memory_order_relaxed); }
  ~BusyGuard() { if (ok) { g_active_calls[m->device & 63].fetch_sub(1, std::memory_order_relaxed); m->busy.clear(std::memory_order_release); } }
};
#define WIS_ENTER(m, what)                                                                                      \
  BusyGuard _busy(m);                                                                                           \
  if (!_busy.ok) { set_error(what ": another call is running on this handle (one call at a time per replica)"); return WIS_E_STATE; }

}

extern "C" {

int wis_version(void) { return WIS_ABI_VERSION; }
const char* wis_last_error(void) { return get_error(); }
int wis_device_count(void) { int n = 0; if (hipGetDeviceCount(&n) != hipSuccess) return 0; return n; }
int wis_supported_compute_types(int device, char* out, size_t cap) {
  (void)device;
  const char* s = "float16,float32,int8_float16";
  if (!out || cap < strlen(s) + 1) { set_error("buffer too small"); return WIS_E_ARG; }
  strcpy(out, s); return WIS_OK;
}

int wis_model_create(const wis_config_t* cfg, const void* arena, size_t arena_bytes, int arena_on_device,
                     const wis_tensor_t* tensors, int n_tensors, int device, wis_model_t** out) {
  if (!cfg || !arena || !tensors || !out || n_tensors <= 0) { set_error("wis_model_create: bad argument"); return WIS_E_ARG; }
  if (cfg->d_model % 128 || cfg->d_model != cfg->n_heads * 64 || cfg->d_model > 2048 || !mel_bins_supported(cfg->n_mels) || cfg->n_enc_layers < 1 || cfg->n_dec_layers < 1 || cfg->n_audio_ctx != 1500 ||
      cfg->n_text_ctx > 512 || cfg->max_batch < 1 || cfg->max_beam < 1 || cfg->max_beam > MAX_R || cfg->n_vocab < 1024) {
    set_error("wis_model_create: unsupported config (d_model %% 128, head_dim 64, n_mels 80 or 128, n_audio_ctx 1500, max_beam <= %d)", MAX_R);
    return WIS_E_UNSUPPORTED;
  }
  DeviceCtx* ctx; WIS_RET(get_ctx(device, &ctx));
  wis_model* m = new wis_model();
  m->cfg = *cfg; m->device = device; m->ctx = ctx;
  m->w8 = cfg->decoder_weight_bits == 8;
  m->cq_fold = !m->w8 && getenv("WIS_NO_CQFOLD") == nullptr;
  m->use_graph = getenv("WIS_NO_GRAPH") == nullptr;
  memset(&m->timing, 0, sizeof(m->timing));
  int rc = WIS_OK;
  void* d_arena = nullptr;
  do {
    if (hipStreamCreateWithFlags(&m->st, hipStreamNonBlocking) != hipSuccess) { set_error("stream create failed"); rc = WIS_E_HIP; break; }
    const char* base = reinterpret_cast<const char*>(arena);
    if (!arena_on_device) {
      if (hipMalloc(&d_arena, arena_bytes) != hipSuccess) { set_error("hipMalloc(arena %zu) failed", arena_bytes); rc = WIS_E_NOMEM; break; }
      if (hipMemcpy(d_arena, arena, arena_bytes, hipMemcpyHostToDevice) != hipSuccess) { set_error("arena upload failed"); rc = WIS_E_HIP; break; }
      base = reinterpret_cast<const char*>(d_arena);
    }
    Loader L{tensors, n_tensors, base, arena_bytes};
    if ((rc = load_weights(m, L))) break;
    {
      std::vector<float> ba(m->n_vocab_pad, 0.f), bb(m->n_vocab_pad, 0.f);
      for (int i = 0; i < cfg->n_suppress; ++i) if (cfg->suppress_ids[i] >= 0 && cfg->suppress_ids[i] < cfg->n_vocab) ba[cfg->suppress_ids[i]] = -INFINITY;
      for (int i = 0; i < cfg->n_suppress_begin; ++i) if (cfg->suppress_ids_begin[i] >= 0 && cfg->suppress_ids_begin[i] < cfg->n_vocab) bb[cfg->suppress_ids_begin[i]] = -INFINITY;
      if ((rc = dalloc(m, &m->bias_all, ba.size())) || (rc = dalloc(m, &m->bias_begin, bb.size()))) break;
      hipMemcpy(m->bias_all, ba.data(), ba.size() * 4, hipMemcpyHostToDevice);
      hipMemcpy(m->bias_begin, bb.data(), bb.size() * 4, hipMemcpyHostToDevice);
      if ((rc = dalloc(m, &m->d_lang_ids, (size_t)(cfg->n_lang > 0 ? cfg->n_lang : 1)))) break;
      if (cfg->n_lang > 0) hipMemcpy(m->d_lang_ids, cfg->lang_ids, (size_t)cfg->n_lang * 4, hipMemcpyHostToDevice);
    }
    m->cfg.suppress_ids = nullptr; m->cfg.suppress_ids_begin = nullptr; m->cfg.lang_ids = nullptr;
    m->wslabs = std::make_shared<WeightSlabs>();
    m->wslabs->device = device; m->wslabs->slabs.swap(m->allocs); m->wslabs->bytes = m->bytes;
    m->slab_cur = nullptr; m->slab_left = 0;
    if ((rc = alloc_buffers(m))) break;
    if (hipStreamSynchronize(m->st) != hipSuccess) { set_error("model init failed"); rc = WIS_E_HIP; break; }
  } while (0);
  if (d_arena) hipFree(d_arena);
  if (rc) { wis_model_destroy(m); return rc; }
  *out = m;
  return WIS_OK;
}

void wis_model_destroy(wis_model_t* m) {
  if (!m) return;
  hipSetDevice(m->device);
  if (m->st) hipStreamSynchronize(m->st);
  spin_collect(m->device);
  for (auto& kv : m->graphs) hipGraphExecDestroy(kv.second);
  for (void* p : m->allocs) hipFree(p);
  if (m->h_pin) hipHostFree(m->h_pin);
  if (m->h_prog) hipHostFree(m->h_prog);
  for (int i = 0; i < 8; ++i) if (m->ev[i]) hipEventDestroy(m->ev[i]);
  for (hipEvent_t e : m->al.ev) if (e) hipEventDestroy(e);
  if (m->st_enc) { hipStreamSynchronize(m->st_enc); hipStreamDestroy(m->st_enc); }
  if (m->ev_enc) hipEventDestroy(m->ev_enc);
  if (m->ev_ckv) hipEventDestroy(m->ev_ckv);
  if (m->st) hipStreamDestroy(m->st);
  delete m;
}
size_t wis_model_device_bytes(const wis_model_t* m) { return m ? m->bytes : 0; }

int wis_model_clone(wis_model_t* parent, wis_model_t** out) {
  if (!parent || !out || !parent->wslabs) { set_error("wis_model_clone: bad argument"); return WIS_E_ARG; }
  WIS_HIP_CHECK(hipSetDevice(parent->device));
  wis_model* m = new wis_model();
  m->cfg = parent->cfg; m->device = parent->device; m->ctx = parent->ctx;
  m->wslabs = parent->wslabs;
  m->w_conv1 = parent->w_conv1; m->w_conv2 = parent->w_conv2; m->b_conv1 = parent->b_conv1; m->b_conv2 = parent->b_conv2;
  m->enc_pos = parent->enc_pos; m->enc_ln_g = parent->enc_ln_g; m->enc_ln_b = parent->enc_ln_b;
  m->enc = parent->enc; m->dec = parent->dec;
  m->emb = parent->emb; m->dec_pos = parent->dec_pos; m->p_proj = parent->p_proj; m->dec_ln_g = parent->dec_ln_g; m->dec_ln_b = parent->dec_ln_b;
  m->bias_all = parent->bias_all; m->bias_begin = parent->bias_begin; m->d_lang_ids = parent->d_lang_ids; m->n_vocab_pad = parent->n_vocab_pad;
  m->w_ckv_all = parent->w_ckv_all; m->b_ckv_all = parent->b_ckv_all;
  m->s_proj = parent->s_proj; m->c_proj = parent->c_proj; m->b_proj = parent->b_proj; m->w8 = parent->w8; m->cq_fold = parent->cq_fold;
  m->use_graph = parent->use_graph;
  m->al.heads = parent->al.heads;
  memset(&m->timing, 0, sizeof(m->timing));
  int rc = WIS_OK;
  do {
    if (hipStreamCreateWithFlags(&m->st, hipStreamNonBlocking) != hipSuccess) { set_error("stream create failed"); rc = WIS_E_HIP; break; }
    if ((rc = alloc_buffers(m))) break;
    if (hipStreamSynchronize(m->st) != hipSuccess) { set_error("clone init failed"); rc = WIS_E_HIP; break; }
  } while (0);
  if (rc) { wis_model_destroy(m); return rc; }
  *out = m;
  return WIS_OK;
}

}

static int fill_tree_window(const int* hd, int s0, int Rw, int k, int P, std::vector<int>& tok, std::vector<int>& pos, std::vector<int>& slot, std::vector<int>& ls, int* ha) {
  const int Mreal = k * Rw, Mpad = cdiv(Mreal, 16) * 16;
  tok.assign(Mpad, 0); pos.assign(Mpad, 0); slot.assign(Mpad, 0); ls.assign(Mpad, 0);
  for (int t = 0; t < Rw; ++t) for (int j = 0; j < k; ++j) {
    const int s_ = s0 + t, r = t * k + j;
    tok[r] = hd[((s_ - 1) * MAX_R + j) * 2]; pos[r] = P - 1 + s_; slot[r] = j; ls[r] = j;
    int a = j;
    for (int sp = s_; sp >= s0; --sp) { ha[r * ANC_W + (sp - s0)] = a; a = hd[((sp - 1) * MAX_R + a) * 2 + 1]; }
    for (int u = t + 1; u < ANC_W; ++u) ha[r * ANC_W + u] = ha[r * ANC_W + t];
  }
  for (int r = Mreal; r < Mpad; ++r) {
    tok[r] = tok[Mreal - 1]; pos[r] = pos[Mreal - 1]; slot[r] = slot[Mreal - 1]; ls[r] = ls[Mreal - 1];
    for (int u = 0; u < ANC_W; ++u) ha[r * ANC_W + u] = ha[(Mreal - 1) * ANC_W + u];
  }
  return Mpad;
}

static int generate_impl(wis_model_t* m, const float* input, int B, const int32_t* prompt, int P,
                 const wis_gen_opts_t* o, int32_t* out_ids, int32_t* out_len, float* out_score, bool* retry,
                 const int32_t* draft = nullptr, int n_draft = 0, int* accepted = nullptr, const int32_t* draft_org = nullptr) {
  *retry = false;
  if (accepted) *accepted = 0;
  m->nsp_B = 0;
  WIS_HIP_CHECK(hipSetDevice(m->device));
  SpinClaim claim(m, B);
  const wis_config_t& c = m->cfg;
  const int beam = o->beam_size < 1 ? 1 : o->beam_size;
  WIS_RET(check_batch(m, B, beam));
  WIS_RET(check_patience(beam, o->patience));
  if (P < 1 || P > 16 || B * P > MAX_ROWS) { set_error("prompt length %d unsupported (1..16, B*P <= %d)", P, MAX_ROWS); return WIS_E_UNSUPPORTED; }
  int max_new = o->max_new_tokens > 0 ? o->max_new_tokens : std::min(c.n_text_ctx / 2, c.n_text_ctx - P);
  if (max_new > 256) max_new = 256;
  if (P - 1 + max_new > c.n_text_ctx) max_new = c.n_text_ctx - (P - 1);
  for (int i = 0; i < B * P; ++i) if (prompt[i] < 0 || prompt[i] >= c.n_vocab) { set_error("prompt token %d out of range", prompt[i]); return WIS_E_ARG; }
  hipStream_t st = m->st;
  const int ctx = c.n_text_ctx;
  auto t0 = std::chrono::steady_clock::now();

  const int Mrows = B * beam;
  WIS_RET(init_beam_state(m, B, beam));
  float patience;
  const SampleCfg sc = make_sample_cfg(m, o, beam, max_new, &patience);
  const float* bias_all = o->suppress_default ? m->bias_all : nullptr;
  const bool drafting = draft != nullptr && n_draft > 0;
  const bool beam_draft = drafting && draft_org != nullptr;
  if (drafting && B != 1) { set_error("wis_generate_draft: one utterance per call (got B = %d)", B); return WIS_E_UNSUPPORTED; }
  if (drafting && !beam_draft && beam != 1) { set_error("wis_generate_draft: beam_size 1 (a beam search is drafted by its trajectory: wis_generate_draft_beam)"); return WIS_E_UNSUPPORTED; }
  const bool ts = o->timestamps != 0;
  const int ts_max_init = o->max_initial_timestamp_index < 0 ? -1 : o->max_initial_timestamp_index;
  if (ts && draft != nullptr) { set_error("timestamps: not available for drafted decodes (wis_generate_draft / wis_generate_draft_beam)"); return WIS_E_UNSUPPORTED; }
  int sot_row = -1;
  if (o->no_speech_prob && !drafting) {
    for (int i = 0; i < P; ++i) if (prompt[i] == c.sot) { sot_row = i; break; }
    for (int b = 1; b < B && sot_row >= 0; ++b) if (prompt[b * P + sot_row] != c.sot) sot_row = -1;
    if (sot_row < 0) { set_error("no_speech_prob: the prompts hold no common <|startoftranscript|> position"); return WIS_E_ARG; }
  }
  if (beam_draft && (beam < 2 || n_draft > 256)) { set_error("wis_generate_draft_beam: beam_size >= 2 and at most 256 draft steps (got %d, %d)", beam, n_draft); return WIS_E_ARG; }
  if (drafting) for (int i = 0; i < n_draft * (beam_draft ? beam : 1); ++i) if (draft[i] < 0 || draft[i] >= c.n_vocab) { set_error("draft token %d out of range", draft[i]); return WIS_E_ARG; }
  if (beam_draft) for (int i = 0; i < n_draft * beam; ++i) if (draft_org[i] < 0 || draft_org[i] >= beam) { set_error("draft origin %d outside [0, beam_size)", draft_org[i]); return WIS_E_ARG; }
  m->last_B = B; m->last_beam = beam;
  const bool spin_call = m->spin_now;
  if (drafting) m->spin_now = false;
  if (!drafting || beam_draft) {
    std::vector<int> tok(B * P), pos(B * P), slot(B * P), ls(B * P);
    for (int b = 0; b < B; ++b) for (int i = 0; i < P; ++i) { tok[b * P + i] = prompt[b * P + i]; pos[b * P + i] = i; slot[b * P + i] = b * beam; ls[b * P + i] = b * beam; }
    WIS_RET(upload_rows(m, tok, pos, slot, ls, false));
  }
  const unsigned long long gen = m->gen;
  if (m->overrun_left) { WIS_HIP_CHECK(hipMemsetAsync(m->ca_epoch, 0, 4, st)); m->overrun_left = false; }
  __atomic_store_n(&m->h_prog[HP_REC], 0ull, __ATOMIC_RELAXED);
  m->h_prog[HP_DONE_STEP] = 0; m->h_prog[HP_DONE_STAMP] = 0; m->h_prog[HP_STAMP0] = 0;

  static const bool one_stream = getenv("WIS_ONE_STREAM") != nullptr;
  static const bool two_streams = getenv("WIS_TWO_STREAMS") != nullptr;
  const bool alone = g_active_calls[m->device & 63].load(std::memory_order_relaxed) <= 1;
  hipStream_t se = (one_stream || !(alone || two_streams)) ? st : m->st_enc;
  if (se != st) WIS_HIP_CHECK(hipStreamWaitEvent(se, m->ev_ckv, 0));
  WIS_HIP_CHECK(hipEventRecord(m->ev[0], se));
  WIS_RET(stage_input(m, input, o->input_kind, B, se));
  WIS_HIP_CHECK(hipEventRecord(m->ev[1], se));
  WIS_RET(run_encoder(m, B, se));
  WIS_HIP_CHECK(hipEventRecord(m->ev[2], se));
  if (se != st) { WIS_HIP_CHECK(hipEventRecord(m->ev_enc, se)); WIS_HIP_CHECK(hipStreamWaitEvent(st, m->ev_enc, 0)); }
  WIS_RET(run_cross_kv(m, B));
  WIS_HIP_CHECK(hipEventRecord(m->ev[3], st));
  WIS_HIP_CHECK(hipEventRecord(m->ev_ckv, st));

  int steps = 1;
  bool spec_done = false;
  bool beam_fin = false;
  std::vector<int> spec_gen; float spec_cum = 0.f; int spec_len = 0;
  if (!drafting) {
    WIS_RET(dec_forward(m, B * P, P, B, true, beam, 0));
    if (sot_row >= 0) WIS_RET(launch_no_speech(st, m->logits, m->n_vocab_pad, B, P, sot_row, c.n_vocab, c.no_speech, m->d_nsp));
    if (ts) WIS_RET(launch_ts_rules(st, m->logits, bias_all, m->bias_begin, m->bs, B, sc, c.no_timestamps, ts_max_init, P, 0, P - 1, m->ts_desc));
    WIS_RET(launch_logit_stats(st, m->logits, bias_all, m->bias_begin, m->bs.step_u, m->st_max, m->st_sum, m->st_val, m->st_idx, B, sc, P, 0, P - 1, WIS_TAPS ? m->d_prof + (size_t)m->cfg.n_dec_layers * 8 * 16 + 16 : nullptr,
                               nullptr, ts ? m->ts_desc : nullptr));
    WIS_RET(launch_beam_step(st, m->st_max, m->st_sum, m->st_val, m->st_idx, m->bs, m->rm, B, P, ctx, sc, WIS_TAPS ? m->d_prof + (size_t)m->cfg.n_dec_layers * 8 * 16 : nullptr));
    WIS_RET(launch_kv_reorder(st, m->kc_all, m->vc_all, m->kv_layer_stride, c.n_dec_layers, m->bs, B, beam, P, ctx, c.d_model));
  } else if (beam_draft) {
    const int k = beam;
    const int nd = std::min(n_draft, max_new - 1);
    int* hd = m->h_pin + 8192;
    for (int s_ = 0; s_ < nd; ++s_) for (int j = 0; j < k; ++j) { hd[(s_ * MAX_R + j) * 2] = draft[s_ * k + j]; hd[(s_ * MAX_R + j) * 2 + 1] = draft_org[s_ * k + j]; }
    int* hv = m->h_pin + 12288;
    for (int i = 0; i < 32; ++i) hv[i] = 0;
    for (int j = 0; j < MAX_R; ++j) { hv[DRAFT_VS_PERM + j] = j; hv[DRAFT_VS_BASE + j] = j; }
    if (nd > 0) WIS_HIP_CHECK(hipMemcpyAsync(m->d_draft, hd, (size_t)nd * MAX_R * 2 * 4, hipMemcpyHostToDevice, st));
    WIS_HIP_CHECK(hipMemcpyAsync(m->d_vstate, hv, 32 * 4, hipMemcpyHostToDevice, st));
    WIS_RET(dec_forward(m, P, P, 1, true, beam, 0));
    WIS_RET(launch_logit_stats(st, m->logits, bias_all, m->bias_begin, m->bs.step_u, m->st_max, m->st_sum, m->st_val, m->st_idx, 1, sc, P, 0, P - 1));
    WIS_RET(launch_beam_step(st, m->st_max, m->st_sum, m->st_val, m->st_idx, m->bs, m->rm, 1, P, ctx, sc));
    WIS_RET(launch_kv_reorder(st, m->kc_all, m->vc_all, m->kv_layer_stride, c.n_dec_layers, m->bs, 1, beam, P, ctx, c.d_model));
    WIS_RET(launch_draft_match(st, m->bs, m->d_draft, nd, k, m->d_vstate, 0));
    const int RW = std::min(ANC_W, MAX_ROWS / k);
    const int s_last = std::min(nd, max_new - 1);
    int* ha = m->h_pin + 12352;
    int* hb = m->h_pin + 15872;
    int* hw2 = m->h_pin + 16000;
    int done_flag = 0, step_dev = 0;
    int pinv[MAX_R];
    for (int j = 0; j < MAX_R; ++j) pinv[j] = j;
    for (int s0 = 1;; ) {
      const int Rw = std::min(RW, s_last - s0 + 1);
      if (Rw >= 1) {
        std::vector<int> tok, pos, slot, ls;
        const int Mpad = fill_tree_window(hd, s0, Rw, k, P, tok, pos, slot, ls, ha);
        for (int r = 0; r < Mpad; ++r) hb[r] = pinv[ha[r * ANC_W]];
        const RowMeta rm_search = m->rm;
        m->rm = m->rm_win;
        int rc = upload_rows(m, tok, pos, slot, ls, false, 15488);
        if (!rc && (hipMemcpyAsync(m->d_anc, ha, (size_t)Mpad * ANC_W * 4, hipMemcpyHostToDevice, st) != hipSuccess ||
                    hipMemcpyAsync(m->d_base, hb, (size_t)Mpad * 4, hipMemcpyHostToDevice, st) != hipSuccess)) { set_error("draft window: ancestor table upload failed"); rc = WIS_E_HIP; }
        TreeWin tw{m->d_anc, P - 1 + s0, ANC_W}; tw.base = m->d_base;
        if (!rc) rc = dec_forward(m, Mpad, 16, Mpad / 16, true, 1, 0, &tw);
        m->rm = rm_search;
        WIS_RET(rc);
        hw2[0] = 0; for (int j = 0; j < MAX_R; ++j) hw2[1 + j] = j;
        WIS_HIP_CHECK(hipMemcpyAsync(m->d_vstate + 2, hw2, 4, hipMemcpyHostToDevice, st));
        WIS_HIP_CHECK(hipMemcpyAsync(m->d_vstate + DRAFT_VS_BASE, hw2 + 1, MAX_R * 4, hipMemcpyHostToDevice, st));
        for (int t = 0; t < Rw; ++t) {
          WIS_RET(launch_logit_stats(st, m->logits, bias_all, m->bias_begin, m->bs.step_u, m->st_max, m->st_sum, m->st_val, m->st_idx, 1, sc, beam, 1, t * k, nullptr, m->d_vstate + DRAFT_VS_PERM));
          WIS_RET(launch_beam_step(st, m->st_max, m->st_sum, m->st_val, m->st_idx, m->bs, m->rm, 1, P, ctx, sc));
          WIS_RET(launch_draft_match(st, m->bs, m->d_draft, nd, k, m->d_vstate, 1));
        }
        WIS_RET(launch_kv_gather(st, m->kc_all, m->vc_all, m->kv_layer_stride, c.n_dec_layers, m->d_vstate, m->bs.done, beam, P - 1 + s0, ctx, c.d_model));
      }
      WIS_HIP_CHECK(hipMemcpyAsync(hv, m->d_vstate, 16 * 4, hipMemcpyDeviceToHost, st));
      WIS_HIP_CHECK(hipMemcpyAsync(hv + 24, m->bs.done, 4, hipMemcpyDeviceToHost, st));
      WIS_HIP_CHECK(hipMemcpyAsync(hv + 25, m->bs.step_u, 4, hipMemcpyDeviceToHost, st));
      WIS_HIP_CHECK(hipStreamSynchronize(st));
      done_flag = hv[24]; step_dev = hv[25];
      if (Rw < 1 || done_flag != 0) break;
      for (int j = 0; j < k; ++j) { const int n_ = hv[DRAFT_VS_PERM + j]; if (n_ >= 0 && n_ < k) pinv[n_] = j; }
      s0 += Rw;
    }
    if (accepted) *accepted = hv[0];
    __atomic_store_n(&m->h_prog[HP_REC], 0ull, __ATOMIC_RELAXED);
    if (done_flag == 1) {
      beam_fin = true; steps = step_dev + 1;
    } else {
      steps = step_dev;
      if (steps < 1) { set_error("wis_generate_draft_beam: verification completed no step"); return WIS_E_STATE; }
      int* hw = m->h_pin + 4096 + 512;
      unsigned* tk = reinterpret_cast<unsigned*>(hw);
      tk[0] = (unsigned)steps; tk[1] = m->gen; tk[2] = 0; tk[3] = 0;
      WIS_HIP_CHECK(hipMemcpyAsync(m->bs.tick, tk, 16, hipMemcpyHostToDevice, st));
      WIS_HIP_CHECK(hipMemsetAsync(m->bs.done, 0, 4, st));
    }
  } else {
    const int nd = std::min(n_draft, max_new - 1);
    std::vector<int> seq(P + nd);
    for (int i = 0; i < P; ++i) seq[i] = prompt[i];
    for (int i = 0; i < nd; ++i) seq[P + i] = draft[i];
    static const int env_rows = getenv("WIS_DRAFT_ROWS") ? atoi(getenv("WIS_DRAFT_ROWS")) : 0;
    const int R = (env_rows >= 16 && env_rows <= MAX_ROWS) ? env_rows / 16 * 16 : MAX_ROWS;
    bool stop = false; int n_acc = 0;
    for (int t0 = 0; t0 < P + nd && !stop; t0 += R) {
      const int rows = std::min(R, P + nd - t0);
      const int f = std::max(P - 1 - t0, 0), nv = rows - f;
      const int Mp = rows > 16 ? cdiv(rows, 16) * 16 : rows;
      std::vector<int> tok(Mp), pos(Mp), slot(Mp, 0), ls(Mp, 0);
      for (int i = 0; i < Mp; ++i) { const int ii = std::min(i, rows - 1); tok[i] = seq[t0 + ii]; pos[i] = t0 + ii; }
      WIS_RET(upload_rows(m, tok, pos, slot, ls));
      if (rows > 16) {
        WIS_HIP_CHECK(hipMemsetAsync(m->d_anc, 0, (size_t)Mp * 16 * 4, st));
        const TreeWin tw{m->d_anc, t0, 16};
        WIS_RET(dec_forward(m, Mp, 16, Mp / 16, nv > 0, 1, 0, &tw));
      } else
      WIS_RET(dec_forward(m, rows, rows, 1, nv > 0, 1, 0));
      if (nv <= 0) continue;
      int* hv = m->h_pin + 4096;
      for (int i = 0; i < nv; ++i) hv[i] = t0 + f + i - (P - 1);
      WIS_HIP_CHECK(hipMemcpyAsync(m->vstep, hv, (size_t)nv * 4, hipMemcpyHostToDevice, st));
      WIS_RET(launch_logit_stats(st, m->logits, bias_all, m->bias_begin, m->vstep, m->st_max, m->st_sum, m->st_val, m->st_idx, nv, sc, 1, 0, f));
      WIS_RET(launch_greedy_pick(st, m->st_max, m->st_sum, m->st_val, m->st_idx, nv, sc, m->pick_tok, m->pick_lp));
      int* ht = m->h_pin + 4096 + MAX_ROWS; float* hl = reinterpret_cast<float*>(m->h_pin + 4096 + 2 * MAX_ROWS);
      WIS_HIP_CHECK(hipMemcpyAsync(ht, m->pick_tok, (size_t)nv * 4, hipMemcpyDeviceToHost, st));
      WIS_HIP_CHECK(hipMemcpyAsync(hl, m->pick_lp, (size_t)nv * 4, hipMemcpyDeviceToHost, st));
      WIS_HIP_CHECK(hipStreamSynchronize(st));
      for (int i = 0; i < nv && !stop; ++i) {
        const int g = hv[i];
        spec_cum = hl[i] + spec_cum;
        spec_gen.push_back(ht[i]);
        const bool eos = ht[i] == c.eot, is_last = g + 1 >= max_new;
        if (eos || is_last) { spec_done = true; spec_len = eos ? g : g + 1; stop = true; }
        else if (g < nd && ht[i] == draft[g]) ++n_acc;
        else stop = true;
      }
    }
    if (accepted) *accepted = n_acc;
    steps = (int)spec_gen.size();
    if (steps < 1) { set_error("wis_generate_draft: verification produced no token"); return WIS_E_STATE; }
    if (!spec_done) {
      int* hs = m->h_pin + 4096;
      for (int t = 0; t < steps; ++t) hs[t] = spec_gen[t];
      WIS_HIP_CHECK(hipMemcpyAsync(m->bs.alive, hs, (size_t)steps * 4, hipMemcpyHostToDevice, st));
      int* hw = m->h_pin + 4096 + 512;
      hw[0] = steps; hw[1] = spec_gen.back(); hw[2] = P - 1 + steps; hw[3] = 0;
      memcpy(hw + 4, &spec_cum, 4);
      WIS_HIP_CHECK(hipMemcpyAsync(m->bs.step_u, hw, 4, hipMemcpyHostToDevice, st));
      WIS_HIP_CHECK(hipMemcpyAsync(m->rm.tok, hw + 1, 4, hipMemcpyHostToDevice, st));
      WIS_HIP_CHECK(hipMemcpyAsync(m->rm.pos, hw + 2, 4, hipMemcpyHostToDevice, st));
      WIS_HIP_CHECK(hipMemcpyAsync(m->rm.slot, hw + 3, 4, hipMemcpyHostToDevice, st));
      WIS_HIP_CHECK(hipMemcpyAsync(m->rm.lslot, hw + 3, 4, hipMemcpyHostToDevice, st));
      WIS_HIP_CHECK(hipMemcpyAsync(m->bs.cum, hw + 4, 4, hipMemcpyHostToDevice, st));
      unsigned* tk = reinterpret_cast<unsigned*>(hw + 8);
      tk[0] = (unsigned)steps; tk[1] = m->gen; tk[2] = 0; tk[3] = 0;
      WIS_HIP_CHECK(hipMemcpyAsync(m->bs.tick, tk, 16, hipMemcpyHostToDevice, st));
    }
  }
  m->spin_now = spin_call;
  WIS_HIP_CHECK(hipEventRecord(m->ev[4], st));
  if (beam_fin) WIS_HIP_CHECK(hipEventRecord(m->ev[5], st));

  auto one_step = [&]() -> int {
    WIS_RET(dec_forward(m, Mrows, beam, B, true, beam, 1));
    if (ts) WIS_RET(launch_ts_rules(st, m->logits, bias_all, m->bias_begin, m->bs, B, sc, c.no_timestamps, ts_max_init, beam, 1, 0, m->ts_desc));
    WIS_RET(launch_logit_stats(st, m->logits, bias_all, m->bias_begin, m->bs.step_u, m->st_max, m->st_sum, m->st_val, m->st_idx, B, sc, beam, 1, 0, WIS_TAPS ? m->d_prof + (size_t)m->cfg.n_dec_layers * 8 * 16 + 16 : nullptr,
                               nullptr, ts ? m->ts_desc : nullptr));
    WIS_RET(launch_beam_step(st, m->st_max, m->st_sum, m->st_val, m->st_idx, m->bs, m->rm, B, P, ctx, sc, WIS_TAPS ? m->d_prof + (size_t)m->cfg.n_dec_layers * 8 * 16 : nullptr));
    WIS_RET(launch_kv_reorder(st, m->kc_all, m->vc_all, m->kv_layer_stride, c.n_dec_layers, m->bs, B, beam, P, ctx, c.d_model));
    return WIS_OK;
  };
  static const bool sa_short = !(getenv("WIS_SA_NB") && atoi(getenv("WIS_SA_NB")) == 0);
  auto nb_for = [&](int passes_done) { const int len = P + passes_done; return !sa_short ? 8 : (len <= 16 ? 2 : (len <= 32 ? 4 : 8)); };
  struct NbReset { wis_model* m; ~NbReset() { m->sa_nb = 8; } } nb_reset{m};
  auto graph_for = [&](int nb, hipGraphExec_t* out) -> int {
    GraphKey key; memset(&key, 0, sizeof(key));
    key.B = B; key.beam = beam; key.P = P; key.max_new = max_new; key.fixed_new = sc.fixed_new; key.suppress_blank = sc.suppress_blank;
    key.suppress_default = o->suppress_default; key.early_exit = sc.allow_early_exit; key.lp = sc.length_penalty; key.patience = patience; key.spin = (m->spin_now ? 1 : 0) | (sa_fuse_enabled() ? 2 : 0);
    key.sa_nb = nb;
    key.timestamps = ts ? 1 : 0; key.max_init = ts ? ts_max_init : 0;
    auto it = m->graphs.find(key);
    if (it != m->graphs.end()) { *out = it->second; return WIS_OK; }
    hipGraph_t graph = nullptr; hipGraphExec_t ge = nullptr;
    WIS_HIP_CHECK(hipStreamBeginCapture(st, hipStreamCaptureModeThreadLocal));
    int rc = one_step();
    hipError_t e = hipStreamEndCapture(st, &graph);
    if (rc) { if (graph) hipGraphDestroy(graph); return rc; }
    if (e != hipSuccess) { set_error("graph capture failed: %s", hipGetErrorString(e)); return WIS_E_HIP; }
    e = hipGraphInstantiate(&ge, graph, nullptr, nullptr, 0);
    hipGraphDestroy(graph);
    if (e != hipSuccess) { set_error("graph instantiate failed: %s", hipGetErrorString(e)); return WIS_E_HIP; }
    m->graphs[key] = ge;
    *out = ge;
    return WIS_OK;
  };
  auto launch_pass = [&](int passes_done) -> int {
    m->sa_nb = nb_for(passes_done);
    if (!m->use_graph) return one_step();
    hipGraphExec_t ge = nullptr;
    WIS_RET(graph_for(m->sa_nb, &ge));
    WIS_HIP_CHECK(hipGraphLaunch(ge, st));
    return WIS_OK;
  };
  int needed = 0;
  bool gave_up = false, from_host = false;
  float decode_ms_dev = -1.f;
  const int known = (sc.fixed_new > 0) ? std::min(max_new, sc.fixed_new + 1) : 0;
  const int limit = known ? known : max_new;
  auto unpack = [&](unsigned long long r, int* st_, int* dn_, int* gu_) {
    if ((r >> 48) != gen) { *st_ = 0; *dn_ = 0; *gu_ = 0; return; }
    *st_ = (int)((r >> 32) & 0xFFFFu); *gu_ = (int)((r >> 16) & 0xFFFFu); *dn_ = (int)(r & 0xFFFFu);
  };
  const int base_done = drafting ? steps : 0;
  const auto t_dec0 = std::chrono::steady_clock::now();
  if (spec_done || beam_fin) {
    needed = steps;
  } else if (known) {
    for (; steps < limit; ++steps) WIS_RET(launch_pass(steps));
    WIS_HIP_CHECK(hipEventRecord(m->ev[5], st));
    WIS_HIP_CHECK(hipStreamSynchronize(st));
    int st_, dn_, gu_; unpack(__atomic_load_n(&m->h_prog[HP_REC], __ATOMIC_ACQUIRE), &st_, &dn_, &gu_);
    gave_up = gu_ != 0;
    if (!gave_up && dn_ < B) { set_error("decode did not terminate within %d steps (done %d of %d)", steps, dn_, B); return WIS_E_STATE; }
    needed = steps;
  } else {
    const int depth = o->queue_depth > 0 ? o->queue_depth : 2;
    auto t_last = std::chrono::steady_clock::now();
    int seen = -1, st_ = 0, dn_ = 0, gu_ = 0;
    static const bool trace = getenv("WIS_EOT_TRACE") != nullptr;
    struct Tr { int step; unsigned long long dev; double host_us; int launched; };
    std::vector<Tr> tr;
    const auto t_loop = std::chrono::steady_clock::now();
    for (unsigned spins = 0;; ++spins) {
      unpack(__atomic_load_n(&m->h_prog[HP_REC], __ATOMIC_ACQUIRE), &st_, &dn_, &gu_);
      if (st_ < base_done) st_ = base_done;
      if (dn_ >= B || gu_) break;
      if (st_ >= limit) break;
      if (steps < limit && steps - st_ < depth) {
        const auto tl0 = std::chrono::steady_clock::now();
        WIS_RET(launch_pass(steps));
        ++steps;
        if (trace) tr.push_back({-steps, 0ull, std::chrono::duration<double, std::micro>(std::chrono::steady_clock::now() - tl0).count(), steps});
        continue;
      }
      if (st_ != seen) {
        seen = st_; t_last = std::chrono::steady_clock::now(); spins = 0;
        if (trace) tr.push_back({st_, m->h_prog[HP_STAMP], std::chrono::duration<double, std::micro>(t_last - t_loop).count(), steps});
      }
      else if ((spins & 1023u) == 1023u) {
        const double idle = std::chrono::duration<double>(std::chrono::steady_clock::now() - t_last).count();
        if (idle > 30.0) { set_error("decode made no progress for 30 s (step %d of %d enqueued)", st_, steps); return WIS_E_HIP; }
        if (idle > 200e-6) { struct timespec ts = {0, 20000}; nanosleep(&ts, nullptr); }
      }
      cpu_relax();
    }
    if (trace) {
      unsigned long long prev_dev = 0;
      for (size_t i = 0; i < tr.size(); ++i) {
        if (tr[i].step < 0) { fprintf(stderr, "[eot-trace]   launch of step %d took the host %.1f us\n", -tr[i].step, tr[i].host_us); continue; }
        fprintf(stderr, "[eot-trace] step %d seen by the host at %.1f us (device clock +%.1f us since the previous record), %d steps enqueued\n", tr[i].step, tr[i].host_us,
                prev_dev ? (double)(tr[i].dev - prev_dev) * 0.01 : 0.0, tr[i].launched);
        prev_dev = tr[i].dev;
      }
      fprintf(stderr, "[eot-trace] done seen at %.1f us: %d of %d utterances, %d steps enqueued\n", std::chrono::duration<double, std::micro>(std::chrono::steady_clock::now() - t_loop).count(), dn_, B, steps);
    }
    gave_up = gu_ != 0;
    if (!gave_up && dn_ < B) { set_error("decode did not terminate within %d steps (done %d of %d)", steps, dn_, B); return WIS_E_STATE; }
    if (!gave_up) {
      from_host = true;
      needed = (int)m->h_prog[HP_DONE_STEP];
      const unsigned long long s0 = m->h_prog[HP_STAMP0], s1 = m->h_prog[HP_DONE_STAMP];
      decode_ms_dev = s1 > s0 ? (float)((double)(s1 - s0) * 1e-5) : 0.f;
      if (drafting) decode_ms_dev = std::chrono::duration<float, std::milli>(std::chrono::steady_clock::now() - t_dec0).count();
    }
  }
  if (gave_up) {
    WIS_HIP_CHECK(hipMemsetAsync(m->ca_epoch, 0, 4, st));
    WIS_HIP_CHECK(hipStreamSynchronize(st));
    m->spin_off = true; *retry = true; ++m->handoff_retries;
    fprintf(stderr, "[wis_hip] device %d: decoder cross-attention granule hand-off timed out; this handle uses the ticket hand-off from now on, the call is repeated\n", m->device);
    return WIS_OK;
  }
  if (spec_done) {
    float sfin = spec_cum;
    if (sc.length_penalty != 0.f) sfin /= powf((float)spec_len, sc.length_penalty);
    out_len[0] = spec_len;
    for (int t = 0; t < max_new; ++t) out_ids[t] = t < spec_len ? spec_gen[t] : 0;
    if (out_score) out_score[0] = sfin;
    from_host = true; decode_ms_dev = 0.f;
  } else if (from_host) {
    const int* hl = hp_out_len(m->h_prog); const float* hs = hp_out_score(m->h_prog); const int* hi = hp_out_ids(m->h_prog);
    for (int b = 0; b < B; ++b) {
      int n = hl[b];
      if (n < 0 || n > max_new) { set_error("decode result of utterance %d has length %d outside [0, %d]", b, n, max_new); return WIS_E_STATE; }
      out_len[b] = n;
      for (int t = 0; t < max_new; ++t) out_ids[(size_t)b * max_new + t] = t < n ? hi[(size_t)b * max_new + t] : 0;
      if (out_score) out_score[b] = hs[b];
    }
  } else {
    std::vector<int32_t> ids((size_t)B * 256);
    WIS_HIP_CHECK(hipMemcpyAsync(ids.data(), m->bs.out_ids, (size_t)B * 256 * 4, hipMemcpyDeviceToHost, st));
    WIS_HIP_CHECK(hipMemcpyAsync(out_len, m->bs.out_len, (size_t)B * 4, hipMemcpyDeviceToHost, st));
    std::vector<float> sc_h(B);
    WIS_HIP_CHECK(hipMemcpyAsync(sc_h.data(), m->bs.out_score, (size_t)B * 4, hipMemcpyDeviceToHost, st));
    WIS_HIP_CHECK(hipStreamSynchronize(st));
    for (int b = 0; b < B; ++b) {
      if (out_len[b] > max_new) out_len[b] = max_new;
      for (int t = 0; t < max_new; ++t) out_ids[(size_t)b * max_new + t] = t < out_len[b] ? ids[(size_t)b * max_new + t] : 0;
      if (out_score) out_score[b] = sc_h[b];
    }
  }
  auto t1 = std::chrono::steady_clock::now();
  float ms;
  hipEventElapsedTime(&ms, m->ev[0], m->ev[1]); m->timing.logmel_ms = ms;
  hipEventElapsedTime(&ms, m->ev[1], m->ev[2]); m->timing.encoder_ms = ms;
  hipEventElapsedTime(&ms, m->ev[2], m->ev[3]); m->timing.crosskv_ms = ms;
  hipEventElapsedTime(&ms, m->ev[3], m->ev[4]); m->timing.prefill_ms = ms;
  if (from_host) m->timing.decode_ms = decode_ms_dev; else { hipEventElapsedTime(&ms, m->ev[4], m->ev[5]); m->timing.decode_ms = ms; }
  m->timing.total_ms = std::chrono::duration<float, std::milli>(t1 - t0).count();
  m->timing.decode_steps = steps;
  m->timing.decode_steps_needed = needed;
  if (steps > needed) { claim.defer(st); m->overrun_left = true; }
  if (sot_row >= 0) m->nsp_B = B;
  return WIS_OK;
}

extern "C" {

int wis_generate(wis_model_t* m, const float* input, int B, const int32_t* prompt, int P,
                 const wis_gen_opts_t* o, int32_t* out_ids, int32_t* out_len, float* out_score) {
  if (!m || !input || !prompt || !o || !out_ids || !out_len) { set_error("wis_generate: bad argument"); return WIS_E_ARG; }
  WIS_ENTER(m, "wis_generate")
  bool retry = false;
  WIS_RET(generate_impl(m, input, B, prompt, P, o, out_ids, out_len, out_score, &retry));
  if (retry) {
    WIS_RET(generate_impl(m, input, B, prompt, P, o, out_ids, out_len, out_score, &retry));
    if (retry) { set_error("wis_generate: hand-off flag raised without the granule path"); return WIS_E_STATE; }
  }
  return WIS_OK;
}

int wis_generate_draft(wis_model_t* m, const float* input, const int32_t* prompt, int P, const wis_gen_opts_t* o,
                       const int32_t* draft, int n_draft, int32_t* out_ids, int32_t* out_len, float* out_score, int32_t* accepted) {
  if (!m || !input || !prompt || !o || !out_ids || !out_len || (n_draft > 0 && !draft) || n_draft < 0) { set_error("wis_generate_draft: bad argument"); return WIS_E_ARG; }
  if (o->timestamps) { set_error("wis_generate_draft: timestamps are not available for drafted decodes"); return WIS_E_UNSUPPORTED; }
  WIS_ENTER(m, "wis_generate_draft")
  bool retry = false;
  int acc = 0;
  WIS_RET(generate_impl(m, input, 1, prompt, P, o, out_ids, out_len, out_score, &retry, draft, n_draft, &acc));
  if (retry) {
    WIS_RET(generate_impl(m, input, 1, prompt, P, o, out_ids, out_len, out_score, &retry, draft, n_draft, &acc));
    if (retry) { set_error("wis_generate_draft: hand-off flag raised without the granule path"); return WIS_E_STATE; }
  }
  if (accepted) *accepted = acc;
  return WIS_OK;
}

int wis_generate_draft_beam(wis_model_t* m, const float* input, const int32_t* prompt, int P, const wis_gen_opts_t* o,
                            const int32_t* draft_tok, const int32_t* draft_org, int n_steps, int32_t* out_ids, int32_t* out_len, float* out_score, int32_t* accepted_steps) {
  if (!m || !input || !prompt || !o || !out_ids || !out_len || n_steps < 0 || (n_steps > 0 && (!draft_tok || !draft_org))) { set_error("wis_generate_draft_beam: bad argument"); return WIS_E_ARG; }
  if (o->timestamps) { set_error("wis_generate_draft_beam: timestamps are not available for drafted decodes"); return WIS_E_UNSUPPORTED; }
  WIS_ENTER(m, "wis_generate_draft_beam")
  bool retry = false;
  int acc = 0;
  for (int attempt = 0; attempt < 2; ++attempt) {
    WIS_RET(generate_impl(m, input, 1, prompt, P, o, out_ids, out_len, out_score, &retry, n_steps > 0 ? draft_tok : nullptr, n_steps, &acc, n_steps > 0 ? draft_org : nullptr));
    if (!retry) break;
    if (attempt == 1) { set_error("wis_generate_draft_beam: hand-off flag raised without the granule path"); return WIS_E_STATE; }
  }
  if (accepted_steps) *accepted_steps = acc;
  return WIS_OK;
}

int wis_last_no_speech_prob(wis_model_t* m, int B, float* out) {
  if (!m || !out || B < 1) { set_error("wis_last_no_speech_prob: bad argument"); return WIS_E_ARG; }
  WIS_ENTER(m, "wis_last_no_speech_prob")
  if (m->nsp_B == 0) { set_error("wis_last_no_speech_prob: the last wis_generate on this handle did not ask for no_speech_prob"); return WIS_E_STATE; }
  if (B > m->nsp_B) { set_error("wis_last_no_speech_prob: %d utterances asked, the last call had %d", B, m->nsp_B); return WIS_E_ARG; }
  WIS_HIP_CHECK(hipSetDevice(m->device));
  WIS_HIP_CHECK(hipMemcpyAsync(out, m->d_nsp, (size_t)B * 4, hipMemcpyDeviceToHost, m->st));
  WIS_HIP_CHECK(hipStreamSynchronize(m->st));
  return WIS_OK;
}

int wis_last_trajectory(wis_model_t* m, int b, int32_t* tok, int32_t* org, int cap_steps, int32_t* n_steps) {
  if (!m || !tok || !org || !n_steps || cap_steps < 0) { set_error("wis_last_trajectory: bad argument"); return WIS_E_ARG; }
  WIS_ENTER(m, "wis_last_trajectory")
  WIS_HIP_CHECK(hipSetDevice(m->device));
  if (b < 0 || b >= m->last_B) { set_error("wis_last_trajectory: utterance %d outside the last call's batch of %d", b, m->last_B); return WIS_E_ARG; }
  const int k = m->last_beam;
  int n = 0;
  WIS_HIP_CHECK(hipMemcpyAsync(&n, m->bs.step_u + b, 4, hipMemcpyDeviceToHost, m->st));
  WIS_HIP_CHECK(hipStreamSynchronize(m->st));
  if (n < 0 || n > 256) { set_error("wis_last_trajectory: step counter %d out of range", n); return WIS_E_STATE; }
  if (n > cap_steps) n = cap_steps;
  std::vector<int> raw((size_t)n * MAX_R * 2);
  if (n) WIS_HIP_CHECK(hipMemcpy(raw.data(), m->bs.traj + (size_t)b * 256 * MAX_R * 2, raw.size() * 4, hipMemcpyDeviceToHost));
  for (int s = 0; s < n; ++s) for (int j = 0; j < k; ++j) { tok[s * k + j] = raw[((size_t)s * MAX_R + j) * 2]; org[s * k + j] = raw[((size_t)s * MAX_R + j) * 2 + 1]; }
  *n_steps = n;
  return WIS_OK;
}

int wis_debug_search(wis_model_t* m, const float* logits, int n_steps, int B, const wis_gen_opts_t* o,
                     int32_t* out_ids, int32_t* out_len, float* out_score, int32_t* out_finish_step, int32_t* out_parent) {
  if (!m || !logits || !o || !out_ids || !out_len || n_steps < 1 || n_steps > 256) { set_error("wis_debug_search: bad argument"); return WIS_E_ARG; }
  WIS_ENTER(m, "wis_debug_search")
  WIS_HIP_CHECK(hipSetDevice(m->device));
  const wis_config_t& c = m->cfg;
  const int beam = o->beam_size < 1 ? 1 : o->beam_size;
  WIS_RET(check_batch(m, B, beam));
  WIS_RET(check_patience(beam, o->patience));
  const int max_new = o->max_new_tokens > 0 ? std::min(o->max_new_tokens, 256) : n_steps;
  if (max_new > n_steps) { set_error("wis_debug_search: %d steps of logits for max_new_tokens %d", n_steps, max_new); return WIS_E_ARG; }
  hipStream_t st = m->st;
  const int Mrows = B * beam, V = c.n_vocab, P = 1;
  WIS_RET(init_beam_state(m, B, beam));
  float patience;
  const SampleCfg sc = make_sample_cfg(m, o, beam, max_new, &patience);
  const float* bias_all = o->suppress_default ? m->bias_all : nullptr;
  const bool ts = o->timestamps != 0;
  const int ts_max_init = o->max_initial_timestamp_index < 0 ? -1 : o->max_initial_timestamp_index;
  std::vector<int> done(B, 0), fin(B, -1), par(Mrows);
  for (int s = 0; s < max_new; ++s) {
    WIS_HIP_CHECK(hipMemcpy2DAsync(m->logits, (size_t)m->n_vocab_pad * 4, logits + (size_t)s * Mrows * V, (size_t)V * 4, (size_t)V * 4, Mrows, hipMemcpyHostToDevice, st));
    if (ts) WIS_RET(launch_ts_rules(st, m->logits, bias_all, m->bias_begin, m->bs, B, sc, c.no_timestamps, ts_max_init, beam, s == 0 ? 0 : 1, 0, m->ts_desc));
    WIS_RET(launch_logit_stats(st, m->logits, bias_all, m->bias_begin, m->bs.step_u, m->st_max, m->st_sum, m->st_val, m->st_idx, B, sc, beam, s == 0 ? 0 : 1, 0, nullptr, nullptr,
                               ts ? m->ts_desc : nullptr));
    WIS_RET(launch_beam_step(st, m->st_max, m->st_sum, m->st_val, m->st_idx, m->bs, m->rm, B, P, c.n_text_ctx, sc));
    WIS_HIP_CHECK(hipMemcpyAsync(done.data(), m->bs.done, (size_t)B * 4, hipMemcpyDeviceToHost, st));
    WIS_HIP_CHECK(hipMemcpyAsync(par.data(), m->bs.parent, (size_t)Mrows * 4, hipMemcpyDeviceToHost, st));
    WIS_HIP_CHECK(hipStreamSynchronize(st));
    bool all = true;
    for (int b = 0; b < B; ++b) { if (done[b] && fin[b] < 0) fin[b] = s; all = all && done[b]; }
    if (out_parent) for (int r = 0; r < Mrows; ++r) out_parent[(size_t)s * Mrows + r] = par[r];
    if (all) break;
  }
  for (int b = 0; b < B; ++b) if (fin[b] < 0) { set_error("wis_debug_search: utterance %d did not finish within %d steps", b, max_new); return WIS_E_STATE; }
  std::vector<int32_t> ids((size_t)B * 256);
  std::vector<float> sc_h(B);
  WIS_HIP_CHECK(hipMemcpyAsync(ids.data(), m->bs.out_ids, (size_t)B * 256 * 4, hipMemcpyDeviceToHost, st));
  WIS_HIP_CHECK(hipMemcpyAsync(out_len, m->bs.out_len, (size_t)B * 4, hipMemcpyDeviceToHost, st));
  WIS_HIP_CHECK(hipMemcpyAsync(sc_h.data(), m->bs.out_score, (size_t)B * 4, hipMemcpyDeviceToHost, st));
  WIS_HIP_CHECK(hipStreamSynchronize(st));
  for (int b = 0; b < B; ++b) {
    if (out_len[b] > max_new) out_len[b] = max_new;
    for (int t = 0; t < max_new; ++t) out_ids[(size_t)b * max_new + t] = t < out_len[b] ? ids[(size_t)b * max_new + t] : 0;
    if (out_score) out_score[b] = sc_h[b];
    if (out_finish_step) out_finish_step[b] = fin[b];
  }
  return WIS_OK;
}

int wis_debug_handoff(wis_model_t* m, int raise_flag, int* retries, int* spin_disabled) {
  if (!m) { set_error("wis_debug_handoff: bad argument"); return WIS_E_ARG; }
  WIS_ENTER(m, "wis_debug_handoff")
  WIS_HIP_CHECK(hipSetDevice(m->device));
  if (raise_flag) {
    const unsigned one = 1u;
    WIS_HIP_CHECK(hipMemcpyAsync(m->ca_epoch, &one, 4, hipMemcpyHostToDevice, m->st));
    WIS_HIP_CHECK(hipStreamSynchronize(m->st));
  }
  if (retries) *retries = m->handoff_retries;
  if (spin_disabled) *spin_disabled = m->spin_off ? 1 : 0;
  return WIS_OK;
}

int wis_last_timing(const wis_model_t* m, wis_timing_t* t) {
  if (!m || !t) { set_error("wis_last_timing: bad argument"); return WIS_E_ARG; }
  *t = m->timing; return WIS_OK;
}

static int single_row_setup(wis_model* m, int B, const std::vector<int>& tok, int pos) {
  const int ctx = m->cfg.n_text_ctx;
  std::vector<int> ps(B, pos), slot(B), ls(B);
  for (int r = 0; r < B; ++r) { slot[r] = r; ls[r] = r; }
  return upload_rows(m, tok, ps, slot, ls);
}

int wis_detect_language(wis_model_t* m, const float* input, int input_kind, int B, float* lang_probs) {
  if (!m || !input || !lang_probs) { set_error("wis_detect_language: bad argument"); return WIS_E_ARG; }
  if (m->cfg.n_lang <= 0) { set_error("model has no lang_ids"); return WIS_E_UNSUPPORTED; }
  WIS_ENTER(m, "wis_detect_language")
  WIS_HIP_CHECK(hipSetDevice(m->device));
  WIS_RET(check_batch(m, B, 1));
  WIS_RET(stage_input(m, input, input_kind, B));
  WIS_RET(run_encoder(m, B));
  WIS_RET(run_cross_kv(m, B));
  std::vector<int> tok(B, m->cfg.sot);
  for (int attempt = 0; attempt < 2; ++attempt) {
    SpinClaim claim(m, B);
    WIS_RET(single_row_setup(m, B, tok, 0));
    WIS_RET(dec_forward(m, B, 1, B, true, 1, 0));
    WIS_RET(launch_lang_probs(m->st, m->logits, m->n_vocab_pad, m->d_lang_ids, m->cfg.n_lang, m->d_probs, B));
    WIS_HIP_CHECK(hipMemcpyAsync(lang_probs, m->d_probs, (size_t)B * m->cfg.n_lang * 4, hipMemcpyDeviceToHost, m->st));
    bool gave_up = false;
    WIS_RET(spin_gave_up(m, &gave_up));
    if (!gave_up) break;
  }
  return WIS_OK;
}

int wis_debug_encode(wis_model_t* m, const float* input, int input_kind, int B, float* enc_out) {
  if (!m || !input || !enc_out) { set_error("wis_debug_encode: bad argument"); return WIS_E_ARG; }
  WIS_ENTER(m, "wis_debug_encode")
  WIS_HIP_CHECK(hipSetDevice(m->device));
  WIS_RET(check_batch(m, B, 1));
  WIS_RET(stage_input(m, input, input_kind, B));
  WIS_RET(run_encoder(m, B));
  const int64_t n = (int64_t)B * m->cfg.n_audio_ctx * m->cfg.d_model;
  hipLaunchKernelGGL(f16_to_f32_kernel, dim3(blocks_for(n)), dim3(256), 0, m->st, m->mem, m->x, n);
  WIS_HIP_CHECK(hipMemcpyAsync(enc_out, m->x, (size_t)n * 4, hipMemcpyDeviceToHost, m->st));
  WIS_HIP_CHECK(hipStreamSynchronize(m->st));
  return WIS_OK;
}

int wis_debug_logits(wis_model_t* m, const float* input, int input_kind, int B, const int32_t* dec_in, int T, float* logits) {
  if (!m || !input || !dec_in || !logits || T < 1 || T > m->cfg.n_text_ctx) { set_error("wis_debug_logits: bad argument"); return WIS_E_ARG; }
  WIS_ENTER(m, "wis_debug_logits")
  WIS_HIP_CHECK(hipSetDevice(m->device));
  WIS_RET(check_batch(m, B, 1));
  WIS_RET(stage_input(m, input, input_kind, B));
  WIS_RET(run_encoder(m, B));
  WIS_RET(run_cross_kv(m, B));
  const int V = m->cfg.n_vocab;
  for (int t = 0; t < T; ++t) {
    std::vector<int> tok(B);
    for (int b = 0; b < B; ++b) tok[b] = dec_in[b * T + t];
    for (int attempt = 0; attempt < 2; ++attempt) {
      SpinClaim claim(m, B);
      WIS_RET(single_row_setup(m, B, tok, t));
      WIS_RET(dec_forward(m, B, 1, B, true, 1, 0));
      for (int b = 0; b < B; ++b)
        WIS_HIP_CHECK(hipMemcpyAsync(logits + ((size_t)b * T + t) * V, m->logits + (size_t)b * m->n_vocab_pad, (size_t)V * 4, hipMemcpyDeviceToHost, m->st));
      bool gave_up = false;
      WIS_RET(spin_gave_up(m, &gave_up));
      if (!gave_up) break;
    }
  }
  return WIS_OK;
}

int wis_debug_logits_rows(wis_model_t* m, const float* input, int input_kind, int B, const int32_t* dec_in, int T, int R, float* logits) {
  if (!m || !input || !dec_in || !logits || T < 1 || T > m->cfg.n_text_ctx || R < 1 || R > 16) { set_error("wis_debug_logits_rows: bad argument (1 <= R <= 16)"); return WIS_E_ARG; }
  WIS_ENTER(m, "wis_debug_logits_rows")
  WIS_HIP_CHECK(hipSetDevice(m->device));
  WIS_RET(check_batch(m, B, 1));
  if (B * R > MAX_ROWS) { set_error("wis_debug_logits_rows: B*R = %d exceeds %d decoder rows per pass", B * R, MAX_ROWS); return WIS_E_STATE; }
  WIS_RET(stage_input(m, input, input_kind, B));
  WIS_RET(run_encoder(m, B));
  WIS_RET(run_cross_kv(m, B));
  const int V = m->cfg.n_vocab;
  for (int t0 = 0; t0 < T; t0 += R) {
    const int rows = std::min(R, T - t0), M = B * rows;
    std::vector<int> tok(M), pos(M), slot(M), ls(M);
    for (int b = 0; b < B; ++b) for (int i = 0; i < rows; ++i) { const int r = b * rows + i; tok[r] = dec_in[b * T + t0 + i]; pos[r] = t0 + i; slot[r] = b; ls[r] = b; }
    for (int r = 0; r < M; ++r) if (tok[r] < 0 || tok[r] >= V) { set_error("wis_debug_logits_rows: token %d out of range", tok[r]); return WIS_E_ARG; }
    for (int attempt = 0; attempt < 2; ++attempt) {
      SpinClaim claim(m, B);
      WIS_RET(upload_rows(m, tok, pos, slot, ls));
      WIS_RET(dec_forward(m, M, rows, B, true, 1, 0));
      for (int b = 0; b < B; ++b) for (int i = 0; i < rows; ++i)
        WIS_HIP_CHECK(hipMemcpyAsync(logits + ((size_t)b * T + t0 + i) * V, m->logits + (size_t)(b * rows + i) * m->n_vocab_pad, (size_t)V * 4, hipMemcpyDeviceToHost, m->st));
      bool gave_up = false;
      WIS_RET(spin_gave_up(m, &gave_up));
      if (!gave_up) break;
    }
  }
  return WIS_OK;
}

int wis_debug_tree_logits(wis_model_t* m, const float* input, int input_kind, const int32_t* prompt, int P, int beam,
                          const int32_t* tok, const int32_t* org, int n_steps, float* logits) {
  if (!m || !input || !prompt || !tok || !org || !logits || P < 1 || P > 16 || beam < 1 || beam > MAX_R || n_steps < 1 || n_steps > std::min(32, MAX_ROWS / std::max(beam, 1))) {
    set_error("wis_debug_tree_logits: bad argument (1 <= n_steps <= min(32, %d / beam))", MAX_ROWS); return WIS_E_ARG;
  }
  WIS_ENTER(m, "wis_debug_tree_logits")
  WIS_HIP_CHECK(hipSetDevice(m->device));
  WIS_RET(check_batch(m, 1, beam));
  const wis_config_t& c = m->cfg; hipStream_t st = m->st;
  const int k = beam, V = c.n_vocab;
  for (int i = 0; i < n_steps * k; ++i) if (tok[i] < 0 || tok[i] >= V || org[i] < 0 || org[i] >= k) { set_error("wis_debug_tree_logits: token / origin out of range"); return WIS_E_ARG; }
// ... 388 lines not shown
```

Baseline: 147.3 x realtime.

## Merge per-wave candidate lists in logit stats and fuse step embedding into beam step

Adds an optional in-block merge so logit_stats writes one top-candidate list per block (16 lists) rather than one per wave (64 lists), which shrinks the candidate pool that beam_step and greedy_pick have to scan. It also adds a tail to beam_step that computes the next step's token-plus-position embedding rows directly, so the decoder forward can skip its separate embed launch for small beams. The list merge is off by default (tail_merge=false) and the embedding tail is on by default, which adds a graph-key field and gives beam_step extra work per step.

```diff
diff --git a/willow-inference-server_amd/csrc/dec_kernels.hip b/willow-inference-server_amd/csrc/dec_kernels.hip
--- a/willow-inference-server_amd/csrc/dec_kernels.hip
+++ b/willow-inference-server_amd/csrc/dec_kernels.hip
@@ -2121,7 +2121,7 @@
 __device__ __forceinline__ bool better_b(float av, int ai, float bv, int bi) { return (av > bv) | ((av == bv) & (ai < bi)); }
 __device__ __forceinline__ void take_better(float& v, int& i, float ov, int oi) { const bool t = better_b(ov, oi, v, i); v = t ? ov : v; i = t ? oi : i; }
 
-template <bool TS>
+template <bool TS, bool MERGE>
 __global__ __launch_bounds__(256) void logit_stats_kernel(const float* __restrict__ logits, const float* __restrict__ bias_all,
                                                           const float* __restrict__ bias_begin, const int* __restrict__ step_u,
                                                           float* __restrict__ st_max, float* __restrict__ st_sum,
@@ -2129,6 +2129,7 @@
                                                           int lr_b, int lr_j, int lr_off, unsigned long long* prof, const int* __restrict__ rowmap,
                                                           const int* __restrict__ ts_desc) {
   constexpr int PT = 16;
+  __shared__ u64 wk[MERGE ? 4 * MAX_CAND : 1];
   const int tid = threadIdx.x, lane = tid & 63, wave = tid >> 6;
   const int sc = blockIdx.x * 4 + wave, m = blockIdx.y, b = m / cfg.beam;
   unsigned long long* pf = (blockIdx.x == 0 && blockIdx.y == 0 && tid == 0) ? prof : nullptr;
@@ -2187,21 +2188,43 @@
       for (int i = 0; i < w; ++i) t[i] = key_max(t[i], t[i + w]);
     const u64 best = wave_max_key(t[0]);
     if (lane == 0) {
-      st_val[((size_t)m * STAT_SUB + sc) * cfg.n_cand + rnd] = best ? key_value(best) : -INFINITY;
-      st_idx[((size_t)m * STAT_SUB + sc) * cfg.n_cand + rnd] = best ? key_index(best) : 0x7fffffff;
+      if constexpr (MERGE) wk[wave * cfg.n_cand + rnd] = best;
+      else {
+        st_val[((size_t)m * STAT_SUB + sc) * cfg.n_cand + rnd] = best ? key_value(best) : -INFINITY;
+        st_idx[((size_t)m * STAT_SUB + sc) * cfg.n_cand + rnd] = best ? key_index(best) : 0x7fffffff;
+      }
     }
     prev = best;
+  }
+  if constexpr (MERGE) {
+    const int NC = cfg.n_cand;
+    __syncthreads();
+    if (tid < 4 * NC) {
+      const u64 mine = wk[tid];
+      int rank = 0;
+#pragma unroll
+      for (int m2 = 0; m2 < 4 * MAX_CAND; ++m2) {
+        const u64 o = wk[m2 < 4 * NC ? m2 : 0];
+        rank += (m2 < 4 * NC && ((o > mine) | ((o == mine) & (m2 < tid)))) ? 1 : 0;
+      }
+      if (rank < NC) {
+        st_val[((size_t)m * STAT_GRP + blockIdx.x) * NC + rank] = mine ? key_value(mine) : -INFINITY;
+        st_idx[((size_t)m * STAT_GRP + blockIdx.x) * NC + rank] = mine ? key_index(mine) : 0x7fffffff;
+      }
+    }
   }
   stamp(pf, 3);
 }
 int launch_logit_stats(hipStream_t st, const float* logits, const float* bias_all, const float* bias_begin, const int* step_u,
                        float* st_max, float* st_sum, float* st_val, int* st_idx, int B, const SampleCfg& cfg, int lr_b, int lr_j, int lr_off,
-                       unsigned long long* prof, const int* rowmap, const int* ts_desc) {
+                       unsigned long long* prof, const int* rowmap, const int* ts_desc, int lists) {
   if (cdiv(cfg.n_vocab, STAT_SUB) > 16 * 64) { set_error("logit_stats: vocab too large"); return WIS_E_UNSUPPORTED; }
-  if (ts_desc) hipLaunchKernelGGL(logit_stats_kernel<true>, dim3(STAT_SUB / 4, B * cfg.beam), dim3(256), 0, st, logits, bias_all, bias_begin, step_u,
-                                  st_max, st_sum, st_val, st_idx, cfg, lr_b, lr_j, lr_off, prof, rowmap, ts_desc);
-  else hipLaunchKernelGGL(logit_stats_kernel<false>, dim3(STAT_SUB / 4, B * cfg.beam), dim3(256), 0, st, logits, bias_all, bias_begin, step_u,
-                          st_max, st_sum, st_val, st_idx, cfg, lr_b, lr_j, lr_off, prof, rowmap, nullptr);
+  if ((lists != STAT_SUB && lists != STAT_GRP) || cfg.n_cand > MAX_CAND) { set_error("logit_stats: %d candidate lists of %d per row unsupported", lists, cfg.n_cand); return WIS_E_UNSUPPORTED; }
+#define WIS_LS(TSv, MGv) hipLaunchKernelGGL((logit_stats_kernel<TSv, MGv>), dim3(STAT_SUB / 4, B * cfg.beam), dim3(256), 0, st, logits, bias_all, bias_begin, step_u, \
+                                            st_max, st_sum, st_val, st_idx, cfg, lr_b, lr_j, lr_off, prof, rowmap, ts_desc)
+  if (lists == STAT_GRP) { if (ts_desc) WIS_LS(true, true); else WIS_LS(false, true); }
+  else { if (ts_desc) WIS_LS(true, false); else WIS_LS(false, false); }
+#undef WIS_LS
   return WIS_OK;
 }
 
@@ -2307,20 +2330,21 @@
 }
 
 __global__ __launch_bounds__(64) void greedy_pick_kernel(const float* __restrict__ st_max, const float* __restrict__ st_sum, const float* __restrict__ st_val,
-                                                         const int* __restrict__ st_idx, int n_cand, int V, int* __restrict__ tok_out, float* __restrict__ lp_out) {
-  const int m = blockIdx.x, lane = threadIdx.x;
+                                                         const int* __restrict__ st_idx, int n_cand, int V, int* __restrict__ tok_out, float* __restrict__ lp_out, int lists) {
+  const int m = blockIdx.x, lane = threadIdx.x, cl = lane < lists ? lane : lists - 1;
   const float smx = st_max[m * STAT_SUB + lane], ssm = st_sum[m * STAT_SUB + lane];
-  const float v = st_val[((size_t)m * STAT_SUB + lane) * n_cand];
-  const int ix = st_idx[((size_t)m * STAT_SUB + lane) * n_cand];
+  const float v = st_val[((size_t)m * lists + cl) * n_cand];
+  const int ix = st_idx[((size_t)m * lists + cl) * n_cand];
   const float M_ = wave_max(smx);
   const float S = wave_sum(smx > -INFINITY ? ssm * __expf(smx - M_) : 0.f);
   const float lse = M_ + logf(S);
   const int tk = ix > V - 1 ? V - 1 : ix;
-  const u64 best = wave_max_key(sel_key(v > -INFINITY ? v - lse : -INFINITY, tk));
+  const u64 best = wave_max_key(lane < lists ? sel_key(v > -INFINITY ? v - lse : -INFINITY, tk) : 0ull);
   if (lane == 0) { tok_out[m] = key_index(best); lp_out[m] = key_value(best); }
 }
-int launch_greedy_pick(hipStream_t st, const float* st_max, const float* st_sum, const float* st_val, const int* st_idx, int rows, const SampleCfg& cfg, int* tok_out, float* lp_out) {
-  hipLaunchKernelGGL(greedy_pick_kernel, dim3(rows), dim3(64), 0, st, st_max, st_sum, st_val, st_idx, cfg.n_cand, cfg.n_vocab, tok_out, lp_out);
+int launch_greedy_pick(hipStream_t st, const float* st_max, const float* st_sum, const float* st_val, const int* st_idx, int rows, const SampleCfg& cfg, int* tok_out, float* lp_out, int lists) {
+  if (lists < 1 || lists > STAT_SUB) { set_error("greedy_pick: %d candidate lists per row", lists); return WIS_E_ARG; }
+  hipLaunchKernelGGL(greedy_pick_kernel, dim3(rows), dim3(64), 0, st, st_max, st_sum, st_val, st_idx, cfg.n_cand, cfg.n_vocab, tok_out, lp_out, lists);
   return WIS_OK;
 }
 
@@ -2345,22 +2369,50 @@
   __hip_atomic_store(bs.host + HP_REC, rec, __ATOMIC_RELEASE, __HIP_MEMORY_SCOPE_SYSTEM);
 }
 
+__device__ __forceinline__ void step_embed_rows(const StepEmbed& se, int r0, int k, const int* s_tok, const int* s_pos) {
+  typedef _Float16 f16x8_t __attribute__((ext_vector_type(8)));
+  const int c8 = se.d >> 3, total = k * c8;
+  for (int c0 = threadIdx.x; c0 < total; c0 += 4 * 256) {
+    f16x8_t a[4], p[4]; int jr[4], ch[4];
+#pragma unroll
+    for (int u = 0; u < 4; ++u) {
+      const int c = c0 + 256 * u, cc = c < total ? c : total - 1;
+      jr[u] = cc / c8; ch[u] = cc - jr[u] * c8;
+      a[u] = *reinterpret_cast<const f16x8_t*>(se.emb + (size_t)s_tok[jr[u]] * se.d + 8 * ch[u]);
+      p[u] = *reinterpret_cast<const f16x8_t*>(se.pos_emb + (size_t)s_pos[jr[u]] * se.d + 8 * ch[u]);
+    }
+#pragma unroll
+    for (int u = 0; u < 4; ++u) {
+      if (c0 + 256 * u < total) {
+        float v[8]; f16x8_t h;
+#pragma unroll
+        for (int i = 0; i < 8; ++i) { v[i] = (float)a[u][i] + (float)p[u][i]; h[i] = (f16)v[i]; }
+        float4* xo = reinterpret_cast<float4*>(se.x + (size_t)(r0 + jr[u]) * se.d + 8 * ch[u]);
+        xo[0] = make_float4(v[0], v[1], v[2], v[3]); xo[1] = make_float4(v[4], v[5], v[6], v[7]);
+        if (se.xh) *reinterpret_cast<f16x8_t*>(se.xh + (size_t)(r0 + jr[u]) * se.d + 8 * ch[u]) = h;
+      }
+    }
+  }
+}
+
 template <int PSL>
 __global__ __launch_bounds__(256) void beam_step_kernel(const float* __restrict__ st_max, const float* __restrict__ st_sum,
                                                         const float* __restrict__ st_val, const int* __restrict__ st_idx,
-                                                        BeamState bs, RowMeta rm, int P, int ctx, SampleCfg cfg, unsigned long long* prof) {
+                                                        BeamState bs, RowMeta rm, int P, int ctx, SampleCfg cfg, unsigned long long* prof,
+                                                        int NL, StepEmbed se) {
   constexpr int HPT = (MAX_R * 256 + 255) / 256;
   __shared__ float lse[MAX_R], s_cum[MAX_R];
   __shared__ float cand_v[MAX_CAND]; __shared__ int cand_word[MAX_CAND]; __shared__ int cand_org[MAX_CAND];
   __shared__ int nb_src[MAX_R]; __shared__ int nb_tok[MAX_R]; __shared__ float nb_cum[MAX_R];
   __shared__ int hyp_src[MAX_R]; __shared__ int hyp_slot[MAX_R]; __shared__ int hyp_n[MAX_R]; __shared__ int n_newhyp;
   __shared__ int s_finished;
+  __shared__ int s_pos[MAX_R];
   __shared__ int sh_alive[MAX_R * 256];
   const int b = blockIdx.x, tid = threadIdx.x, lane = tid & 63, wave = tid >> 6;
   unsigned long long* pf = (b == 0 && tid == 0) ? prof : nullptr;
   stamp(pf, 0);
   const int k = cfg.beam, NC = cfg.n_cand, V = cfg.n_vocab;
-  const int r0 = b * k, per_row = STAT_SUB * NC, total = k * per_row;
+  const int r0 = b * k, per_row = NL * NC, total = k * per_row;
   float pv_[PSL]; int pi_[PSL];
 #pragma unroll
   for (int u = 0; u < PSL; ++u) {
@@ -2385,7 +2437,15 @@
   const int done_b = bs.done[b];
   const int step = bs.step_u[b];
   const int nh0 = bs.n_hyp[b];
-  if (done_b) { if (tid == 0) publish_step(bs); return; }
+  if (done_b) {
+    if (se.emb) {
+      if (tid < k) { nb_tok[tid] = rm.tok[r0 + tid]; s_pos[tid] = rm.pos[r0 + tid]; }
+      __syncthreads();
+      step_embed_rows(se, r0, k, nb_tok, s_pos);
+    }
+    if (tid == 0) publish_step(bs);
+    return;
+  }
 
   stamp(pf, 1);
 #pragma unroll
@@ -2504,6 +2564,11 @@
     const int* src = bs.hyp_tok + ((size_t)b * cfg.max_hyp + best) * cfg.max_new;
     int* hids = hp_out_ids(bs.host) + (size_t)b * cfg.max_new;
     for (int t = tid; t < n; t += 256) { const int v = src[t]; bs.out_ids[(size_t)b * cfg.max_new + t] = v; hids[t] = v; }
+    if (se.emb) {
+      if (tid < k) { nb_tok[tid] = rm.tok[r0 + tid]; s_pos[tid] = rm.pos[r0 + tid]; }
+      __syncthreads();
+      step_embed_rows(se, r0, k, nb_tok, s_pos);
+    }
     __threadfence_system();
     __syncthreads();
     if (tid == 0) { atomicAdd(bs.all_done, 1); publish_step(bs); }
@@ -2525,15 +2590,29 @@
     }
   }
   if (tid == 0) bs.step_u[b] = step + 1;
+  if (se.emb) {
+    if (tid < k) s_pos[tid] = npos;
+    __syncthreads();
+    step_embed_rows(se, r0, k, nb_tok, s_pos);
+  }
   __syncthreads();
   if (tid == 0) publish_step(bs);
   stamp(pf, 8);
 }
 int launch_beam_step(hipStream_t st, const float* st_max, const float* st_sum, const float* st_val, const int* st_idx,
-                     const BeamState& bs, const RowMeta& rm, int B, int P, int ctx, const SampleCfg& cfg, unsigned long long* prof) {
+                     const BeamState& bs, const RowMeta& rm, int B, int P, int ctx, const SampleCfg& cfg, unsigned long long* prof, int lists, const StepEmbed* emb) {
   if (cfg.beam > MAX_R || cfg.n_cand > MAX_CAND || cfg.max_new > 256 || ctx > 512 || cfg.n_vocab > (1 << 20)) { set_error("beam_step: config out of range"); return WIS_E_UNSUPPORTED; }
-  if (cfg.beam * STAT_SUB * cfg.n_cand <= 16 * 256) hipLaunchKernelGGL(beam_step_kernel<16>, dim3(B), dim3(256), 0, st, st_max, st_sum, st_val, st_idx, bs, rm, P, ctx, cfg, prof);
-  else hipLaunchKernelGGL(beam_step_kernel<32>, dim3(B), dim3(256), 0, st, st_max, st_sum, st_val, st_idx, bs, rm, P, ctx, cfg, prof);
+  if (lists != STAT_SUB && lists != STAT_GRP) { set_error("beam_step: %d candidate lists per row unsupported", lists); return WIS_E_UNSUPPORTED; }
+  StepEmbed se; memset(&se, 0, sizeof(se));
+  if (emb) {
+    if (!emb->emb || !emb->pos_emb || !emb->x || emb->d < 8 || emb->d % 8) { set_error("beam_step: embedding tail needs the tables, the rows and d %% 8 == 0"); return WIS_E_ARG; }
+    se = *emb;
+  }
+  const int pool = cfg.beam * lists * cfg.n_cand;
+#define WIS_BS(PSLv) hipLaunchKernelGGL(beam_step_kernel<PSLv>, dim3(B), dim3(256), 0, st, st_max, st_sum, st_val, st_idx, bs, rm, P, ctx, cfg, prof, lists, se)
+  if (lists == STAT_SUB) { if (pool <= 16 * 256) WIS_BS(16); else WIS_BS(32); }
+  else if (pool <= 4 * 256) WIS_BS(4); else WIS_BS(8);
+#undef WIS_BS
   return WIS_OK;
 }
 
diff --git a/willow-inference-server_amd/csrc/kernels.hpp b/willow-inference-server_amd/csrc/kernels.hpp
--- a/willow-inference-server_amd/csrc/kernels.hpp
+++ b/willow-inference-server_amd/csrc/kernels.hpp
@@ -101,11 +101,13 @@
 #define WIS_EARLY_EXIT_NUM_HYPOTHESES 1
 #endif
 constexpr int STAT_SUB = 64;
+constexpr int STAT_GRP = STAT_SUB / 4;
 int launch_logit_stats(hipStream_t st, const float* logits, const float* bias_all, const float* bias_begin, const int* step_u,
                        float* st_max, float* st_sum, float* st_val, int* st_idx, int B, const SampleCfg& cfg,
                        int lr_b, int lr_j, int lr_off, unsigned long long* prof = nullptr,
                        const int* rowmap = nullptr,
-                       const int* ts_desc = nullptr);
+                       const int* ts_desc = nullptr,
+                       int lists = STAT_SUB);
 constexpr int TS_DESC_INTS = 8;
 struct BeamState;
 int launch_ts_rules(hipStream_t st, const float* logits, const float* bias_all, const float* bias_begin, const BeamState& bs, int B,
@@ -140,12 +142,15 @@
 __host__ __device__ inline float* hp_out_score(unsigned long long* hp) { return reinterpret_cast<float*>(hp + HP_WORDS) + HP_MAXB; }
 __host__ __device__ inline int* hp_out_ids(unsigned long long* hp) { return reinterpret_cast<int*>(hp + HP_WORDS) + 2 * HP_MAXB; }
 int launch_kv_reorder(hipStream_t st, f16* kc, f16* vc, size_t layer_stride, int L, const BeamState& bs, int B, int beam, int P, int ctx, int d);
+struct StepEmbed { const f16* emb; const f16* pos_emb; float* x; f16* xh; int d; };
 int launch_beam_step(hipStream_t st, const float* st_max, const float* st_sum, const float* st_val, const int* st_idx,
-                     const BeamState& bs, const RowMeta& rm, int B, int P, int ctx, const SampleCfg& cfg, unsigned long long* prof = nullptr);
+                     const BeamState& bs, const RowMeta& rm, int B, int P, int ctx, const SampleCfg& cfg, unsigned long long* prof = nullptr,
+                     int lists = STAT_SUB, const StepEmbed* emb = nullptr);
 constexpr int DRAFT_VS_INTS = 32 + MAX_R * 32, DRAFT_VS_PERM = 8, DRAFT_VS_BASE = 16;
 int launch_draft_match(hipStream_t st, const BeamState& bs, const int* draft, int n_draft, int beam, int* vstate, int book);
 int launch_kv_gather(hipStream_t st, f16* kc, f16* vc, size_t layer_stride, int L, const int* vstate, const int* done, int beam, int w0, int ctx, int d);
-int launch_greedy_pick(hipStream_t st, const float* st_max, const float* st_sum, const float* st_val, const int* st_idx, int rows, const SampleCfg& cfg, int* tok_out, float* lp_out);
+int launch_greedy_pick(hipStream_t st, const float* st_max, const float* st_sum, const float* st_val, const int* st_idx, int rows, const SampleCfg& cfg, int* tok_out, float* lp_out,
+                       int lists = STAT_SUB);
 int launch_lang_probs(hipStream_t st, const float* logits, int ld, const int* lang_ids, int n_lang, float* probs, int B);
 
 }
diff --git a/willow-inference-server_amd/csrc/model.hip b/willow-inference-server_amd/csrc/model.hip
--- a/willow-inference-server_amd/csrc/model.hip
+++ b/willow-inference-server_amd/csrc/model.hip
@@ -99,6 +99,7 @@
 struct GraphKey {
   int B, beam, P, max_new, fixed_new, suppress_blank, suppress_default, early_exit, spin, sa_nb; float lp, patience;
   int timestamps, max_init;
+  int tail_merge, tail_embed;
   bool operator<(const GraphKey& o) const { return memcmp(this, &o, sizeof(GraphKey)) < 0; }
 };
 
@@ -177,6 +178,8 @@
   wis_timing_t timing;
   std::map<GraphKey, hipGraphExec_t> graphs;
   bool use_graph;
+  bool tail_merge = false, tail_embed = true;
+  bool embed_done = false;
   float* s_proj = nullptr;
   float* c_proj = nullptr; float* b_proj = nullptr;
   bool w8 = false;
@@ -733,7 +736,8 @@
   const bool ln_ok = fold && d % 64 == 0 && M * (d / 8) <= 13 * 256;
   const bool sa_fuse = m->spin_now && sa_fuse_enabled() && rmul == 1 && M <= 8 && !m->w8 && d % 64 == 0 && ctx >= 64 && !m->prof_on;
   const bool lnp = ln_ok && ln_form == 1 && d <= 1280, ln16 = ln_ok && ln_form == 2 && d <= 2048;
-  WIS_RET(launch_dec_embed(st, m->emb, m->dec_pos, m->rm.tok, m->rm.pos, m->dx, M, d, fold ? m->dxh : nullptr, lnp ? m->dstat : nullptr));
+  if (m->embed_done && (lnp || M > 8)) { set_error("dec_forward: the beam step's embedding tail does not cover this route"); return WIS_E_STATE; }
+  if (!m->embed_done) WIS_RET(launch_dec_embed(st, m->emb, m->dec_pos, m->rm.tok, m->rm.pos, m->dx, M, d, fold ? m->dxh : nullptr, lnp ? m->dstat : nullptr));
   for (int l = 0; l < c.n_dec_layers; ++l) {
     const DecLayerW& w = m->dec[l];
     unsigned long long* pr = (m->prof_on && (l == 0 || m->prof_all)) ? m->d_prof + (size_t)l * 8 * 16 : nullptr;
@@ -890,6 +894,11 @@
   strcpy(out, s); return WIS_OK;
 }
 
+static void read_tail_switches(wis_model* m) {
+  auto on = [](const char* name, bool dflt) { const char* e = getenv(name); return e ? atoi(e) != 0 : dflt; };
+  m->tail_merge = on("WIS_TAIL_MERGE", false); m->tail_embed = on("WIS_TAIL_EMBED", true);
+}
+
 int wis_model_create(const wis_config_t* cfg, const void* arena, size_t arena_bytes, int arena_on_device,
                      const wis_tensor_t* tensors, int n_tensors, int device, wis_model_t** out) {
   if (!cfg || !arena || !tensors || !out || n_tensors <= 0) { set_error("wis_model_create: bad argument"); return WIS_E_ARG; }
@@ -904,6 +913,7 @@
   m->w8 = cfg->decoder_weight_bits == 8;
   m->cq_fold = !m->w8 && getenv("WIS_NO_CQFOLD") == nullptr;
   m->use_graph = getenv("WIS_NO_GRAPH") == nullptr;
+  read_tail_switches(m);
   memset(&m->timing, 0, sizeof(m->timing));
   int rc = WIS_OK;
   void* d_arena = nullptr;
@@ -973,6 +983,7 @@
   m->w_ckv_all = parent->w_ckv_all; m->b_ckv_all = parent->b_ckv_all;
   m->s_proj = parent->s_proj; m->c_proj = parent->c_proj; m->b_proj = parent->b_proj; m->w8 = parent->w8; m->cq_fold = parent->cq_fold;
   m->use_graph = parent->use_graph;
+  read_tail_switches(m);
   m->al.heads = parent->al.heads;
   memset(&m->timing, 0, sizeof(m->timing));
   int rc = WIS_OK;
@@ -1048,6 +1059,10 @@
   if (drafting) for (int i = 0; i < n_draft * (beam_draft ? beam : 1); ++i) if (draft[i] < 0 || draft[i] >= c.n_vocab) { set_error("draft token %d out of range", draft[i]); return WIS_E_ARG; }
   if (beam_draft) for (int i = 0; i < n_draft * beam; ++i) if (draft_org[i] < 0 || draft_org[i] >= beam) { set_error("draft origin %d outside [0, beam_size)", draft_org[i]); return WIS_E_ARG; }
   m->last_B = B; m->last_beam = beam;
+  const int lists = m->tail_merge ? STAT_GRP : STAT_SUB;
+  static const bool ln_partials = getenv("WIS_B1_LN") && !strcmp(getenv("WIS_B1_LN"), "partials");
+  const bool emb_tail = m->tail_embed && !drafting && Mrows <= 8 && !ln_partials && !m->al.capture;
+  const StepEmbed step_emb{m->emb, m->dec_pos, m->dx, m->cq_fold ? m->dxh : nullptr, c.d_model};
   const bool spin_call = m->spin_now;
   if (drafting) m->spin_now = false;
   if (!drafting || beam_draft) {
@@ -1084,8 +1099,8 @@
     if (sot_row >= 0) WIS_RET(launch_no_speech(st, m->logits, m->n_vocab_pad, B, P, sot_row, c.n_vocab, c.no_speech, m->d_nsp));
     if (ts) WIS_RET(launch_ts_rules(st, m->logits, bias_all, m->bias_begin, m->bs, B, sc, c.no_timestamps, ts_max_init, P, 0, P - 1, m->ts_desc));
     WIS_RET(launch_logit_stats(st, m->logits, bias_all, m->bias_begin, m->bs.step_u, m->st_max, m->st_sum, m->st_val, m->st_idx, B, sc, P, 0, P - 1, WIS_TAPS ? m->d_prof + (size_t)m->cfg.n_dec_layers * 8 * 16 + 16 : nullptr,
-                               nullptr, ts ? m->ts_desc : nullptr));
-    WIS_RET(launch_beam_step(st, m->st_max, m->st_sum, m->st_val, m->st_idx, m->bs, m->rm, B, P, ctx, sc, WIS_TAPS ? m->d_prof + (size_t)m->cfg.n_dec_layers * 8 * 16 : nullptr));
+                               nullptr, ts ? m->ts_desc : nullptr, lists));
+    WIS_RET(launch_beam_step(st, m->st_max, m->st_sum, m->st_val, m->st_idx, m->bs, m->rm, B, P, ctx, sc, WIS_TAPS ? m->d_prof + (size_t)m->cfg.n_dec_layers * 8 * 16 : nullptr, lists, emb_tail ? &step_emb : nullptr));
     WIS_RET(launch_kv_reorder(st, m->kc_all, m->vc_all, m->kv_layer_stride, c.n_dec_layers, m->bs, B, beam, P, ctx, c.d_model));
   } else if (beam_draft) {
     const int k = beam;
@@ -1098,8 +1113,8 @@
     if (nd > 0) WIS_HIP_CHECK(hipMemcpyAsync(m->d_draft, hd, (size_t)nd * MAX_R * 2 * 4, hipMemcpyHostToDevice, st));
     WIS_HIP_CHECK(hipMemcpyAsync(m->d_vstate, hv, 32 * 4, hipMemcpyHostToDevice, st));
     WIS_RET(dec_forward(m, P, P, 1, true, beam, 0));
-    WIS_RET(launch_logit_stats(st, m->logits, bias_all, m->bias_begin, m->bs.step_u, m->st_max, m->st_sum, m->st_val, m->st_idx, 1, sc, P, 0, P - 1));
-    WIS_RET(launch_beam_step(st, m->st_max, m->st_sum, m->st_val, m->st_idx, m->bs, m->rm, 1, P, ctx, sc));
+    WIS_RET(launch_logit_stats(st, m->logits, bias_all, m->bias_begin, m->bs.step_u, m->st_max, m->st_sum, m->st_val, m->st_idx, 1, sc, P, 0, P - 1, nullptr, nullptr, nullptr, lists));
+    WIS_RET(launch_beam_step(st, m->st_max, m->st_sum, m->st_val, m->st_idx, m->bs, m->rm, 1, P, ctx, sc, nullptr, lists));
     WIS_RET(launch_kv_reorder(st, m->kc_all, m->vc_all, m->kv_layer_stride, c.n_dec_layers, m->bs, 1, beam, P, ctx, c.d_model));
     WIS_RET(launch_draft_match(st, m->bs, m->d_draft, nd, k, m->d_vstate, 0));
     const int RW = std::min(ANC_W, MAX_ROWS / k);
@@ -1129,8 +1144,8 @@
         WIS_HIP_CHECK(hipMemcpyAsync(m->d_vstate + 2, hw2, 4, hipMemcpyHostToDevice, st));
         WIS_HIP_CHECK(hipMemcpyAsync(m->d_vstate + DRAFT_VS_BASE, hw2 + 1, MAX_R * 4, hipMemcpyHostToDevice, st));
         for (int t = 0; t < Rw; ++t) {
-          WIS_RET(launch_logit_stats(st, m->logits, bias_all, m->bias_begin, m->bs.step_u, m->st_max, m->st_sum, m->st_val, m->st_idx, 1, sc, beam, 1, t * k, nullptr, m->d_vstate + DRAFT_VS_PERM));
-          WIS_RET(launch_beam_step(st, m->st_max, m->st_sum, m->st_val, m->st_idx, m->bs, m->rm, 1, P, ctx, sc));
+          WIS_RET(launch_logit_stats(st, m->logits, bias_all, m->bias_begin, m->bs.step_u, m->st_max, m->st_sum, m->st_val, m->st_idx, 1, sc, beam, 1, t * k, nullptr, m->d_vstate + DRAFT_VS_PERM, nullptr, lists));
+          WIS_RET(launch_beam_step(st, m->st_max, m->st_sum, m->st_val, m->st_idx, m->bs, m->rm, 1, P, ctx, sc, nullptr, lists));
           WIS_RET(launch_draft_match(st, m->bs, m->d_draft, nd, k, m->d_vstate, 1));
         }
         WIS_RET(launch_kv_gather(st, m->kc_all, m->vc_all, m->kv_layer_stride, c.n_dec_layers, m->d_vstate, m->bs.done, beam, P - 1 + s0, ctx, c.d_model));
@@ -1182,8 +1197,8 @@
       int* hv = m->h_pin + 4096;
       for (int i = 0; i < nv; ++i) hv[i] = t0 + f + i - (P - 1);
       WIS_HIP_CHECK(hipMemcpyAsync(m->vstep, hv, (size_t)nv * 4, hipMemcpyHostToDevice, st));
-      WIS_RET(launch_logit_stats(st, m->logits, bias_all, m->bias_begin, m->vstep, m->st_max, m->st_sum, m->st_val, m->st_idx, nv, sc, 1, 0, f));
-      WIS_RET(launch_greedy_pick(st, m->st_max, m->st_sum, m->st_val, m->st_idx, nv, sc, m->pick_tok, m->pick_lp));
+      WIS_RET(launch_logit_stats(st, m->logits, bias_all, m->bias_begin, m->vstep, m->st_max, m->st_sum, m->st_val, m->st_idx, nv, sc, 1, 0, f, nullptr, nullptr, nullptr, lists));
+      WIS_RET(launch_greedy_pick(st, m->st_max, m->st_sum, m->st_val, m->st_idx, nv, sc, m->pick_tok, m->pick_lp, lists));
       int* ht = m->h_pin + 4096 + MAX_ROWS; float* hl = reinterpret_cast<float*>(m->h_pin + 4096 + 2 * MAX_ROWS);
       WIS_HIP_CHECK(hipMemcpyAsync(ht, m->pick_tok, (size_t)nv * 4, hipMemcpyDeviceToHost, st));
       WIS_HIP_CHECK(hipMemcpyAsync(hl, m->pick_lp, (size_t)nv * 4, hipMemcpyDeviceToHost, st));
@@ -1224,11 +1239,14 @@
   if (beam_fin) WIS_HIP_CHECK(hipEventRecord(m->ev[5], st));
 
   auto one_step = [&]() -> int {
-    WIS_RET(dec_forward(m, Mrows, beam, B, true, beam, 1));
+    m->embed_done = emb_tail;
+    const int rc_fwd = dec_forward(m, Mrows, beam, B, true, beam, 1);
+    m->embed_done = false;
+    WIS_RET(rc_fwd);
     if (ts) WIS_RET(launch_ts_rules(st, m->logits, bias_all, m->bias_begin, m->bs, B, sc, c.no_timestamps, ts_max_init, beam, 1, 0, m->ts_desc));
     WIS_RET(launch_logit_stats(st, m->logits, bias_all, m->bias_begin, m->bs.step_u, m->st_max, m->st_sum, m->st_val, m->st_idx, B, sc, beam, 1, 0, WIS_TAPS ? m->d_prof + (size_t)m->cfg.n_dec_layers * 8 * 16 + 16 : nullptr,
-                               nullptr, ts ? m->ts_desc : nullptr));
-    WIS_RET(launch_beam_step(st, m->st_max, m->st_sum, m->st_val, m->st_idx, m->bs, m->rm, B, P, ctx, sc, WIS_TAPS ? m->d_prof + (size_t)m->cfg.n_dec_layers * 8 * 16 : nullptr));
+                               nullptr, ts ? m->ts_desc : nullptr, lists));
+    WIS_RET(launch_beam_step(st, m->st_max, m->st_sum, m->st_val, m->st_idx, m->bs, m->rm, B, P, ctx, sc, WIS_TAPS ? m->d_prof + (size_t)m->cfg.n_dec_layers * 8 * 16 : nullptr, lists, emb_tail ? &step_emb : nullptr));
     WIS_RET(launch_kv_reorder(st, m->kc_all, m->vc_all, m->kv_layer_stride, c.n_dec_layers, m->bs, B, beam, P, ctx, c.d_model));
     return WIS_OK;
   };
@@ -1241,6 +1259,7 @@
     key.suppress_default = o->suppress_default; key.early_exit = sc.allow_early_exit; key.lp = sc.length_penalty; key.patience = patience; key.spin = (m->spin_now ? 1 : 0) | (sa_fuse_enabled() ? 2 : 0);
     key.sa_nb = nb;
     key.timestamps = ts ? 1 : 0; key.max_init = ts ? ts_max_init : 0;
+    key.tail_merge = m->tail_merge ? 1 : 0; key.tail_embed = emb_tail ? 1 : 0;
     auto it = m->graphs.find(key);
     if (it != m->graphs.end()) { *out = it->second; return WIS_OK; }
     hipGraph_t graph = nullptr; hipGraphExec_t ge = nullptr;
@@ -1483,12 +1502,13 @@
   const bool ts = o->timestamps != 0;
   const int ts_max_init = o->max_initial_timestamp_index < 0 ? -1 : o->max_initial_timestamp_index;
   std::vector<int> done(B, 0), fin(B, -1), par(Mrows);
+  const int lists = m->tail_merge ? STAT_GRP : STAT_SUB;
   for (int s = 0; s < max_new; ++s) {
     WIS_HIP_CHECK(hipMemcpy2DAsync(m->logits, (size_t)m->n_vocab_pad * 4, logits + (size_t)s * Mrows * V, (size_t)V * 4, (size_t)V * 4, Mrows, hipMemcpyHostToDevice, st));
     if (ts) WIS_RET(launch_ts_rules(st, m->logits, bias_all, m->bias_begin, m->bs, B, sc, c.no_timestamps, ts_max_init, beam, s == 0 ? 0 : 1, 0, m->ts_desc));
     WIS_RET(launch_logit_stats(st, m->logits, bias_all, m->bias_begin, m->bs.step_u, m->st_max, m->st_sum, m->st_val, m->st_idx, B, sc, beam, s == 0 ? 0 : 1, 0, nullptr, nullptr,
-                               ts ? m->ts_desc : nullptr));
-    WIS_RET(launch_beam_step(st, m->st_max, m->st_sum, m->st_val, m->st_idx, m->bs, m->rm, B, P, c.n_text_ctx, sc));
+                               ts ? m->ts_desc : nullptr, lists));
+    WIS_RET(launch_beam_step(st, m->st_max, m->st_sum, m->st_val, m->st_idx, m->bs, m->rm, B, P, c.n_text_ctx, sc, nullptr, lists));
     WIS_HIP_CHECK(hipMemcpyAsync(done.data(), m->bs.done, (size_t)B * 4, hipMemcpyDeviceToHost, st));
     WIS_HIP_CHECK(hipMemcpyAsync(par.data(), m->bs.parent, (size_t)Mrows * 4, hipMemcpyDeviceToHost, st));
     WIS_HIP_CHECK(hipStreamSynchronize(st));
```

After: 147.5 x realtime (median of 6 runs). About the same (+0.1%).
